# mims-harvard/GNNDelete

Measured on AMD Instinct MI355X. Metric: Del-op train iters/sec, higher is better.
Workload: dtype f32; 1 GPU; synth-collab GCN 2-layer, 5.0% IN edge deletion, full-graph Del step (both_layerwise, mse_mean); num_nodes=235868, in_dim=128, hidden_dim=128, out_dim=64, train_edges_undirected=2122296, df_edges=53057, sdf_edges=1602188, spmm_nnz=1838056, S1=178921, S2=188697, hip_graph=True, matrix_products=fp32 matrix instruction (v_mfma_f32_32x32x2_f32), parallelism=single, ranks_seen=1

## Files before the change

### gnndelete_amd/_lib.py

```python
import ctypes
import os
import re

_HERE = os.path.dirname(os.path.abspath(__file__))
LIB_PATH = os.environ.get('GNNDELETE_HIP_LIB') or os.path.join(_HERE, 'lib', 'libgnndelete_hip.so')
HEADER_PATH = os.path.join(os.path.dirname(_HERE), 'include', 'gnndelete_hip.h')

_i32, _i64, _f32, _f64, _p = ctypes.c_int32, ctypes.c_int64, ctypes.c_float, ctypes.c_double, ctypes.c_void_p

ABI_VERSION = 9

PROTOTYPES = {
    'gd_abi_version': (ctypes.c_int, []),
    'gd_last_error_string': (ctypes.c_char_p, []),
    'gd_build_source_hash': (ctypes.c_char_p, []),
    'gd_matrix_split': (ctypes.c_int, []),
    'gd_set_matrix_split': (ctypes.c_int, [ctypes.c_int]),
    'gd_csr_from_coo_workspace': (_i64, [_i32, _i64]),
    'gd_csr_from_coo': (ctypes.c_int, [_p, _p, _i64, _i32, _p, _p, _p, _p, _p, _i64, _p]),
    'gd_gcn_norm_f32': (ctypes.c_int, [_p, _p, _i32, _p, _p]),
    'gd_spmm_csr_f32': (ctypes.c_int, [_p, _p, _p, _p, _i64, _p, _i64, _p, _f32, _i32, _i32, _p]),
    'gd_spmm_csr_balanced_f32': (ctypes.c_int, [_p, _i32, _p, _i32, _p, _p, _p, _i64, _p, _i64, _p, _f32, _p, _p, _i32,
                                                _i32, _i32, _p, _p]),
    'gd_spmm_csr_onepass_f32': (ctypes.c_int, [_p, _i32, _p, _p, _p, _i64, _p, _i64, _p, _f32, _p, _i32, _i32, _i32, _p, _p]),
# ... 6 lines not shown
    'gd_rgcn_conv_f32': (ctypes.c_int, [_p, _p, _p, _p, _p, _p, _i64, _i32, _p, _i32, _i32, _p, _i64, _i32, _i32, _p]),
    'gd_rowpair_loss_f32': (ctypes.c_int, [_i32, _p, _i64, _p, _p, _i64, _p, _i32, _i32, _p, _p, _i64, _p]),
    'gd_random_walk': (ctypes.c_int, [_p, _p, _i32, _p, _i32, _i32, ctypes.c_uint64, _p, _p]),
    'gd_negative_edges': (ctypes.c_int, [_p, _i64, _i64, ctypes.c_uint64, _p, _i64, _p, _i64, _p]),
    'gd_rank_counts_f32': (ctypes.c_int, [_p, _i64, _p, _i64, _p, _p, _p]),
    'gd_subset_rank_workspace': (_i64, [_i64, _i64]),
    'gd_subset_rank_metrics': (ctypes.c_int, [_p, _p, _p, _p, _p, _i64, _i64, _i64, _i64, _i64, _p, _p, _p, _i64, _p]),
    'gd_subset_rank_metrics_drawn': (ctypes.c_int, [_p, _p, _p, _p, ctypes.c_uint64, ctypes.c_uint64, _i64, _i64, _i64, _i64, _p, _p, _p, _i64, _p]),
    'gd_subset_draw': (ctypes.c_int, [ctypes.c_uint64, ctypes.c_uint64, _i64, _i64, _i64, _p, _i64, _p]),
    'gd_rgcn_tile_kl': (ctypes.c_int32, [_i32, _i32, _i32, _i32]),
    'gd_rgcn_pack_weight_f32': (ctypes.c_int, [_p, _i32, _i32, _i32, _i32, _i32, _p, _p]),
    'gd_rgcn_wave_covers': (ctypes.c_int32, [_i32, _i32, _i32]),
    'gd_rgcn_wave_conv_f32': (ctypes.c_int, [_p, _i32, _i32, _p, _i32, _p, _p, _p, _p, _i64, _i32, _p, _i32, _p, _i64, _i32, _i32, _i32, _p]),
    'gd_rgcn_tile_conv_f32': (ctypes.c_int, [_p, _p, _p, _p, _p, _p, _p, _i32, _p, _i64, _i32, _p, _i32, _i32, _p, _i64, _i32,
                                             _i32, _p, _p, _i32, _p, _p]),
    'gd_rgcn_mean_f32': (ctypes.c_int, [_p, _p, _p, _i64, _p, _i64, _i32, _i32, _i32, _p]),
    'gd_gat_aggregate_f32': (ctypes.c_int, [_p, _p, _p, _p, _p, _i64, _p, _i64, _p, _p, _f32, _i32, _i32, _p]),
    'gd_gat_aggregate_bwd_f32': (ctypes.c_int, [_p, _p, _p, _p, _p, _p, _p, _p, _p, _i64, _p, _i64, _p, _i64,
                                                _p, _p, _p, _f32, _i32, _i32, _p]),
    'gd_gat_balanced_scratch': (_i64, [_i32, _i32]),
    'gd_gat_aggregate_balanced_f32': (ctypes.c_int, [_p, _i32, _p, _i32, _i32, _p, _p, _p, _p, _i64, _p, _i64, _p, _p, _p,
                                                     _p, _f32, _i32, _i32, _i32, _p]),
    'gd_gat_edge_grads_balanced_f32': (ctypes.c_int, [_p, _i32, _p, _i32, _p, _p, _p, _p, _p, _p, _i64, _p, _i64, _p,
                                                      _p, _p, _p, _f32, _i32, _i32, _p, _p]),
    'gd_row_dots_f32': (ctypes.c_int, [_p, _i64, _i32, _i32, _p, _p, _p, _p, _p]),
    'gd_gat_transpose_edges_f32': (ctypes.c_int, [_p, _p, _p, _i32, _p, _p, _p]),
    'gd_rank1_add2_f32': (ctypes.c_int, [_p, _i64, _i32, _i32, _p, _p, _p, _p, _p]),
    'gd_segment_sum_f32': (ctypes.c_int, [_p, _p, _p, _i32, _p, _p]),
    'gd_rows_gemm_f32': (ctypes.c_int, [_p, _i64, _p, _i32, _p, _i32, _i32, _i32, _p, _i32, _p, _i64, _p, _p]),
    'gd_rows_gather_gemm_f32': (ctypes.c_int, [_p, _i64, _i64, _p, _i32, _p, _i32, _i32, _p, _i32, _p, _i64, _p]),
    'gd_rows_gemm_wgrad_workspace': (_i64, [_i32, _i32, _i32]),
    'gd_rows_gemm_ws_covers': (ctypes.c_int, [_i32, _i32, _i32]),
    'gd_rows_gemm_accumulate_f32': (ctypes.c_int, [_p, _i64, _p, _i32, _p, _i32, _i32, _i32, _p, _i64, _p]),
    'gd_rows_gemm_select_f32': (ctypes.c_int, [_p, _p, _p, _i64, _p, _i32, _p, _i32, _i32, _i32, _p, _i32, _p, _i64, _p]),
    'gd_rows_gemm_select_chain_covers': (ctypes.c_int, [_i32, _i32, _i32, _i32, _i32]),
    'gd_rows_gemm_select_chain_f32': (ctypes.c_int, [_p, _i64, _p, _i32, _p, _p, _p, _i64, _p, _i64, _p, _i32, _p, _i32, _i32, _i32,
                                                     _p, _i64, _p]),
    'gd_rows_gemm_dots_f32': (ctypes.c_int, [_p, _p, _p, _i64, _p, _i32, _i32, _i32, _p, _i32, _p, _i64, _p, _i32, _p, _p, _p, _p,
                                             _p]),
    'gd_rows_gemm_signs_f32': (ctypes.c_int, [_p, _i64, _p, _i32, _p, _i32, _i32, _i32, _p, _i32, _p, _i64, _p, _p, _p]),
    'gd_rows_gemm_gated_f32': (ctypes.c_int, [_p, _i64, _p, _i32, _p, _i32, _i32, _i32, _p, _p, _i64, _p]),
    'gd_gate_rows_f32': (ctypes.c_int, [_p, _i64, _p, _i32, _p, _i32, _p, _i64, _p]),
    'gd_rows_gemm_gated_rank1_f32': (ctypes.c_int, [_p, _i64, _p, _i32, _p, _i32, _i32, _i32, _p, _p, _p, _p, _p, _p, _i64, _p]),
    'gd_rows_gemm_wgrad_f32': (ctypes.c_int, [_p, _i64, _p, _p, _i64, _p, _p, _p, _i32, _i32, _i32, _p, _i32, _p, _p]),
    'gd_induced_subgraph_workspace': (_i64, [_i32]),
    'gd_induced_subgraph': (ctypes.c_int, [_p, _p, _p, _i32, _p, _i32, _p, _i32, _p, _i64, _p, _p, _p, _p, _p, _p, _p, _p, _p,
                                           _p, _i64, _p]),
    'gd_batch_csr_workspace': (_i64, [_i32, _i64]),
    'gd_batch_csr': (ctypes.c_int, [_p, _p, _i64, _i32, _i32, _p, _p, _p, _p, _p, _p, _p, _p, _i64, _p]),
    'gd_batch_loss_terms_workspace': (_i64, [_i32, _i64]),
    'gd_batch_loss_terms': (ctypes.c_int, [_p, _i64, _p, _i64, _i32, _p, _i32, _i32, _f32, _f32, _p, _p, _p, _p, _p, _i64, _p]),
    'gd_rowpair_mse_workspace': (_i64, [_i32]),
    'gd_rowpair_mse_f32': (ctypes.c_int, [_p, _i64, _p, _i64, _i32, _p, _p, _i32, _p, _p, _p, _p, _i64, _i32,
                                          _p, _p, _p]),
    'gd_rowtarget_mse_workspace': (_i64, [_i32]),
    'gd_rowtarget_mse_f32': (ctypes.c_int, [_p, _i64, _p, _i32, _p, _p, _p, _p, _i32, _p, _i64, _p, _p, _p]),
    'gd_rowtarget_mse_pair_covers': (ctypes.c_int32, [_i32, _i32]),
    'gd_rowtarget_mse_pair_f32': (ctypes.c_int, [_p, _i64, _p, _i32, _p, _p, _p, _p, _i32, _p, _i64, _p, _p, _i64, _p, _i32, _p, _p, _p, _p, _i32, _p, _i64, _p, _p]),
    'gd_gemm_f32_workspace': (_i64, [_i32, _i32, _i32]),
    'gd_gemm_f32': (ctypes.c_int, [_p, _i64, _p, _i32, _p, _i32, _i32, _p, _p, _i64, _p, _p]),
    'gd_edge_dot_f32': (ctypes.c_int, [_p, _i64, _i32, _p, _p, _p, _i64, _p, _i64, _p, _p]),
    'gd_edge_dot_bwd_f32': (ctypes.c_int, [_p, _i64, _i32, _p, _p, _p, _i64, _p, _p, _i64, _p, _i64, _p]),
    'gd_rows_gemm_wgrad_adam_f32': (ctypes.c_int, [_p, _i64, _p, _p, _i64, _p, _p, _p, _i32, _i32, _i32, _p, _i32, _p,
                                                   _p, _p, _p, _p, _f64, _f64, _f64, _f64, _p]),
    'gd_rows_gemm_wgrad_blocks': (_i32, [_i32]),
    'gd_rows_gemm_wgrad_loss_f32': (ctypes.c_int, [_p, _i64, _p, _p, _i64, _p, _p, _p, _p, _p, _p, _i32, _i32, _i32, _p, _i32,
                                                   _p, _p, _p, _p, _p, _p, _f64, _f64, _f64, _f64, _p]),
    'gd_del_loss_bwd_blocks': (_i32, [_i32]),
    'gd_del_loss_bwd_f32': (ctypes.c_int, [_p, _i64, _p, _i32, _p, _i32, _p, _p, _p, _p, _p, _i64, _p, _i64, _p, _p]),
    'gd_del_loss_bwd_wgrad_f32': (ctypes.c_int, [_p, _i64, _p, _i32, _p, _i32, _p, _p, _p, _p, _p, _i64, _p, _i64, _p, _p, _p]),
    'gd_del_loss_bwd_wgrad_parts': (ctypes.c_int32, [_i32, _i32]),
    'gd_del_loss_bwd_wgrad_parts_f32': (ctypes.c_int, [_p, _i64, _p, _i32, _p, _i32, _p, _p, _p, _p, _p, _i64, _p, _i64, _p, _p, _i32, _p]),
    'gd_del_loss_fold_wgrad_covers': (ctypes.c_int32, [_i32, _i32, _i32]),
    'gd_del_loss_fold_wgrad_parts_f32': (ctypes.c_int, [_p, _i64, _p, _i32, _p, _i32, _p, _p, _p, _p, _p, _i64, _p, _i32, _p, _p, _p, _i32, _p]),
    'gd_del1_loss_wgrad_covers': (ctypes.c_int32, [_i32, _i32]),
    'gd_del1_loss_wgrad_parts': (ctypes.c_int32, [_i32]),
    'gd_del1_chain_loss_wgrad_f32': (ctypes.c_int, [_p, _i64, _p, _i32, _p, _i32, _p, _i64, _p, _p, _p, _p, _p, _p, _i64, _i32, _p, _p, _p, _p, _p, _p, _p, _i32, _p]),
    'gd_del1_chain_fold_covers': (ctypes.c_int32, [_i32, _i32, _i32]),
    'gd_del1_chain_fold_loss_wgrad_f32': (ctypes.c_int, [_p, _i64, _p, _i32, _p, _p, _i32, _p, _i64, _p, _p, _p, _p, _p, _p, _i64, _i32, _p, _p,
                                                         _p, _p, _i32, _p]),
    'gd_layer1_fold_f32': (ctypes.c_int, [_p, _p, _p, _p, _p, _p]),
    'gd_step_tail_fold1_f32': (ctypes.c_int, [_p, _p, _i32, _i32, _i32, _p, _p, _p, _p, _p, _p, _p, _p, _p, _i32, _i32, _i32, _p, _p, _p, _p,
                                              _f64, _f64, _f64, _f64, _p, _i32, _p, _i32, _p, _i32, _p, _p, _p, _p]),
    'gd_del1_loss_wgrad_f32': (ctypes.c_int, [_p, _i64, _p, _i32, _p, _i32, _p, _i64, _p, _p, _p, _p, _p, _p, _i64, _p, _p, _i32, _p]),
    'gd_rowtarget_mse_blocks': (_i32, [_i32]),
    'gd_rowfold_loss_blocks': (_i32, [_i32]),
    'gd_rowfold_loss_f32': (ctypes.c_int, [_i32, _p, _i64, _p, _i32, _i32, _p, _p, _p, _p, _i32, _p, _i64, _p, _p]),
    'gd_rowfold_kld_scale_f32': (ctypes.c_int, [_p, _i32, _f32, _f32, _f32, _f32, _p, _p, _i32, _i32, _p, _i64, _p, _p]),
    'gd_loss_finalize_f32': (ctypes.c_int, [_p, _i32, _p, _i32, _p, _p, _i32, _p, _p, _p]),
    'gd_pairs_sigmoid_mse_workspace': (_i64, [_i32, _i32]),
    'gd_pairs_sigmoid_mse_f32': (ctypes.c_int, [_p, _i64, _p, _i32, _i32, _p, _i64, _f32, _p, _p, _p, _p]),
    'gd_edgeprob_dec_workspace': (_i64, [_i64, _i32]),
    'gd_edgeprob_dec_f32': (ctypes.c_int, [_p, _i64, _i64, _i32, _p, _i64, _p, _i64, _i64, _f32, _p, _p, _p, _p, _p, _p, _p]),
    'gd_edge_incidence_workspace': (_i64, [_i64, _i64]),
    'gd_edge_incidence': (ctypes.c_int, [_p, _p, _i64, _i64, _p, _p, _p, _p, _i64, _p]),
    'gd_edge_incidence_fixed_bytes': (_i64, [_i64, _i64]),
    'gd_edge_incidence_fixed': (ctypes.c_int, [_p, _p, _i64, _i64, _p, _i64, _p, _i64, _p]),
    'gd_edge_incidence_update_workspace': (_i64, [_i64, _i64]),
    'gd_edge_incidence_update': (ctypes.c_int, [_p, _p, _p, _i64, _i64, _i64, _p, _p, _p, _p, _i64, _p]),
    'gd_rows_add_f32': (ctypes.c_int, [_p, _i64, _i64, _p, _i32, _p, _i64, _f32, _i32, _p]),
    'gd_edgeprob_record_f32': (ctypes.c_int, [_p, _p, _f32, _f32, _p, _i32, _p, _p]),
    'gd_edgeprob_batch_loss_workspace': (_i64, [_i64, _i64, _i32]),
    'gd_edgeprob_batch_loss_f32': (ctypes.c_int, [_p, _i64, _i64, _p, _i64, _i64, _i32, _p, _i64, _p, _i64, _i64, _p, _p, _i64, _f32, _f32,
                                                  _p, _i64, _p, _p, _p, _p, _p, _p, _p, _i64, _p, _p]),
    'gd_edge_bce_workspace': (_i64, [_i64, _i32]),
    'gd_edge_bce_f32': (ctypes.c_int, [_p, _i64, _i64, _i32, _p, _i64, _i64, _p, _i64, _i64, _f32, _p, _p, _p, _p, _p, _p, _p]),
    'gd_col_sum_workspace': (_i64, [_i64, _i32]),
    'gd_col_sum_f32': (ctypes.c_int, [_p, _i64, _i64, _i32, _p, _p, _p, _p, _p, _p]),
    'gd_row_nll_workspace': (_i64, [_i64, _i32]),
    'gd_row_nll_f32': (ctypes.c_int, [_p, _i64, _i64, _i32, _i32, _p, _i64, _p, _f32, _p, _i64, _p, _p, _p]),
    'gd_eval_edge_scores_workspace': (_i64, [_i64, _i32]),
    'gd_eval_edge_scores_f32': (ctypes.c_int, [_p, _i64, _i64, _i32, _p, _p, _i64, _i64, _i64, _i64, _p, _p, _p, _p, _p]),
    'gd_eval_triple_scores_workspace': (_i64, [_i64, _i32]),
    'gd_eval_triple_scores_f32': (ctypes.c_int, [_p, _i64, _i64, _i32, _p, _i64, _i64, _p, _p, _p, _i64, _i64, _i64, _i64, _p, _p, _p, _p, _p]),
    'gd_row_nll_eval_workspace': (_i64, [_i64, _i32]),
    'gd_row_nll_eval_f32': (ctypes.c_int, [_p, _i64, _i64, _i32, _p, _i64, _p, _p, _p, _p, _p]),
    'gd_adam_at_f32': (ctypes.c_int, [_p, _p, _p, _p, _p, _i64, _f64, _f64, _f64, _f64, _p]),
    'gd_adam_f32': (ctypes.c_int, [_p, _p, _p, _p, _p, _i64, _f64, _f64, _f64, _f64, _p]),
    'gd_segment_softmax_f32': (ctypes.c_int, [_p, _p, _i32, _p, _p]),
    'gd_segment_softmax_bwd_f32': (ctypes.c_int, [_p, _p, _p, _i32, _p, _p]),
    'gd_rowpair_dot_f32': (ctypes.c_int, [_p, _i64, _p, _p, _i64, _p, _i64, _i32, _p, _p]),
    'gd_spmm_csr_onepass_aux_f32': (ctypes.c_int, [_p, _i32, _p, _p, _p, _p, _i64, _p, _i64, _p, _i32, _i32, _i32, _p, _p]),
    'gd_typed_wgrad_f32': (ctypes.c_int, [_p, _i32, _p, _p, _p, _p, _i64, _p, _i64, _i32, _i32, _i32, _p, _p]),
    'gd_typed_edge_dot_f32': (ctypes.c_int, [_p, _p, _p, _i64, _p, _i64, _p, _i64, _p, _i32, _i32, _i32, _p, _p]),
    'gd_comm_unique_id': (ctypes.c_int, [_p]),
    'gd_comm_init': (ctypes.c_int, [_p, _i32, _i32, ctypes.POINTER(ctypes.c_void_p)]),
    'gd_comm_destroy': (ctypes.c_int, [_p]),
    'gd_allreduce_f32': (ctypes.c_int, [_p, _i64, _p, _p]),
    'gd_exchange_rows_f32': (ctypes.c_int, [_p, _p, _p, _p, _i32, _i32, _p, _p]),
}

_lib = None


class GnnDeleteHipError(RuntimeError):
    pass


def declared_symbols():
    with open(HEADER_PATH) as f:
        text = re.sub(r'/\*.*?\*/', '', f.read(), flags=re.S)
    return sorted(set(re.findall(r'\b(gd_[a-z0-9_]+)\s*\(', text)))


def _sources_hash():
    from .source_hash import source_files, source_hash
    return source_hash() if all(os.path.exists(f) for f in source_files()) and os.path.isdir(os.path.join(_HERE, 'csrc')) else None


def build_stamp():
    return lib().gd_build_source_hash().decode(), _sources_hash()


def lib():
    global _lib
    if _lib is None:
        if not os.path.exists(LIB_PATH):
            raise GnnDeleteHipError(
                f'{LIB_PATH} is missing: the HIP extension is not built. Run '
                '`python -c "import __graft_entry__ as g; g.build()"` (or `make -C gnndelete_amd/csrc`). '
                'There is no CPU fallback.')
        import torch
        handle = ctypes.CDLL(LIB_PATH)
        for name, (res, args) in PROTOTYPES.items():
            fn = getattr(handle, name)
            fn.restype, fn.argtypes = res, args
# ... 24 lines not shown
```

### gnndelete_amd/csrc/rows_gemm.hip

```cpp
#include "common.h"

namespace gd {

using f32x16 = __attribute__((ext_vector_type(16))) float;
using bf16x8 = __attribute__((ext_vector_type(8))) __bf16;
using bf16x2 = __attribute__((ext_vector_type(2))) __bf16;
using f32x2 = __attribute__((ext_vector_type(2))) float;
using u32x4v = __attribute__((ext_vector_type(4))) uint32_t;

__device__ inline void split8(const float4 a, const float4 b, bf16x8 (&s)[3]) {
  const f32x2 v[4] = {{a.x, a.y}, {a.z, a.w}, {b.x, b.y}, {b.z, b.w}};
  u32x4v p[3];
#pragma unroll
  for (int i = 0; i < 4; ++i) {
    f32x2 r = v[i];
#pragma unroll
    for (int q = 0; q < 3; ++q) {
      const uint32_t w = __builtin_bit_cast(uint32_t, __builtin_convertvector(r, bf16x2));
      p[q][i] = w;
      if (q < 2) {
        f32x2 h;
        h[0] = __builtin_bit_cast(float, w << 16);
        h[1] = __builtin_bit_cast(float, w & 0xffff0000u);
        r = r - h;
      }
    }
  }
#pragma unroll
  for (int q = 0; q < 3; ++q) s[q] = __builtin_bit_cast(bf16x8, p[q]);
}

constexpr int kWgradMaxRows = 1024;

constexpr int kGemmThreads = 512;

struct RowDots { const float* u1; const float* u2; float* o1; float* o2; };

template <int NT, int MODE, bool SEL = false, int NP = 0, int KC = 0, bool QUEUE = false, bool GATHER = false>
__global__ __launch_bounds__(QUEUE ? 1024 : kGemmThreads, (NP && KC) ? 2 : 4) void rows_gemm_mfma_kernel(
    const float* in, int64_t ld_in, const int32_t* __restrict__ idx, int32_t n_sel,
    const float* __restrict__ w, int32_t d_in, int32_t trans_w, const float* __restrict__ bias, int32_t relu_in,
    float* out, int64_t ld_out, float* __restrict__ save_in, const uint32_t* __restrict__ gate_bits,
    uint32_t* __restrict__ sign_out, const float* in_alt, const uint8_t* __restrict__ sel, RowDots dots,
    const int64_t* __restrict__ gidx, int32_t n_in) {
  static_assert(!GATHER || (MODE == 0 && !SEL && !QUEUE), "the gathering row map is built for the plain product");
  extern __shared__ __attribute__((aligned(16))) float wl[];
  constexpr int d_out = 32 * NT;
  constexpr int kGemmThreads = QUEUE ? 1024 : gd::kGemmThreads;
  constexpr int kWaves = kGemmThreads / 64;
  static_assert(!QUEUE || (NP == 0 && KC == 0), "the tile queue is built for the fp32 form");
  const int tid = threadIdx.x;
  const int lane = tid & 63;
  const int wave = tid >> 6;

  constexpr int NTP = NT == 3 ? 4 : NT;
  bf16x8* const wimg = reinterpret_cast<bf16x8*>(wl);
  const int pstride = (d_in >> 3) * d_out;
  if (NP) {
    for (int e = tid; e < pstride; e += kGemmThreads) {
      const int kg = e / d_out, n = e - kg * d_out;
      float v[8];
#pragma unroll
      for (int c = 0; c < 8; ++c) v[c] = trans_w ? w[(int64_t)n * d_in + 8 * kg + c] : w[(int64_t)(8 * kg + c) * d_out + n];
      bf16x8 pc[3];
      split8(make_float4(v[0], v[1], v[2], v[3]), make_float4(v[4], v[5], v[6], v[7]), pc);
      const int off = ((((kg >> 2) * 2 + (kg & 1)) * NT + (n >> 5)) * 2 + ((kg >> 1) & 1)) * 32 + (n & 31);
#pragma unroll
      for (int q = 0; q < 3; ++q) wimg[q * pstride + off] = pc[q];
    }
  }
  constexpr int kFill = 8;
  for (int e0 = tid; !NP && e0 < d_in * 32; e0 += kGemmThreads * kFill) {
    float v[kFill][NTP];
#pragma unroll
    for (int u = 0; u < kFill; ++u) {
      const int e = min(e0 + u * kGemmThreads, d_in * 32 - 1);
      const int k = e >> 5, r = e & 31;
#pragma unroll
      for (int t = 0; t < NTP; ++t)
        v[u][t] = t < NT ? (trans_w ? w[(int64_t)(32 * t + r) * d_in + k] : w[(int64_t)k * d_out + 32 * t + r]) : 0.f;
    }
#pragma unroll
    for (int u = 0; u < kFill; ++u) {
// ... 499 lines not shown
    float p = 0.f;
    for (int s = s_begin; s < s_end; ++s) {
      const int64_t ra = a_idx ? a_idx[s] : s, rg = g_idx ? g_idx[s] : s;
      float gg = g[rg * ld_g + j];
      if (relu_mask) gg = relu_mask[rg * ld_g + j] > 0.f ? gg : 0.f;
      if (g_add) gg += g_add[rg * ld_g + j];
      p = fmaf(a[ra * ld_a + i], gg, p);
    }
    dst[e] = p;
  }
}

__global__ __launch_bounds__(256) void wgrad_reduce_kernel(const float* __restrict__ partials, int32_t n_part,
                                                           int32_t n_elem, int32_t accumulate,
                                                           float* __restrict__ dw) {
  __shared__ float4 red[16][16];
  const int v = threadIdx.x & 15, slice = threadIdx.x >> 4;
  const int e4 = blockIdx.x * 16 + v;
  const int n4 = n_elem >> 2;
  float4 s0 = f4_zero(), s1 = f4_zero(), s2 = f4_zero(), s3 = f4_zero();
  if (e4 < n4) {
    int b = slice;
    for (; b + 48 < n_part; b += 64) {
      const float4 p0 = reinterpret_cast<const float4*>(partials + (int64_t)b * n_elem)[e4];
      const float4 p1 = reinterpret_cast<const float4*>(partials + (int64_t)(b + 16) * n_elem)[e4];
      const float4 p2 = reinterpret_cast<const float4*>(partials + (int64_t)(b + 32) * n_elem)[e4];
      const float4 p3 = reinterpret_cast<const float4*>(partials + (int64_t)(b + 48) * n_elem)[e4];
      s0 = f4_add(s0, p0); s1 = f4_add(s1, p1); s2 = f4_add(s2, p2); s3 = f4_add(s3, p3);
    }
    for (; b < n_part; b += 16) s0 = f4_add(s0, reinterpret_cast<const float4*>(partials + (int64_t)b * n_elem)[e4]);
  }
  red[slice][v] = f4_add(f4_add(s0, s1), f4_add(s2, s3));
  __syncthreads();
  if (slice == 0 && e4 < n4) {
    float4 t = accumulate ? reinterpret_cast<float4*>(dw)[e4] : f4_zero();
#pragma unroll
    for (int i = 0; i < 16; ++i) t = f4_add(t, red[i][v]);
    reinterpret_cast<float4*>(dw)[e4] = t;
  }
}

__global__ __launch_bounds__(256) void wgrad_reduce_adam_kernel(const float* __restrict__ partials, int32_t n_part,
                                                                int32_t n_elem, int32_t accumulate,
                                                                float* __restrict__ dw, float* __restrict__ param,
                                                                float* __restrict__ m, float* __restrict__ v,
                                                                const int32_t* __restrict__ iter, double lr, double beta1,
                                                                double beta2, double eps) {
  __shared__ float4 red[16][16];
  const int vv = threadIdx.x & 15, slice = threadIdx.x >> 4;
  const int e4 = blockIdx.x * 16 + vv;
  const int n4 = n_elem >> 2;
  float4 s0 = f4_zero(), s1 = f4_zero(), s2 = f4_zero(), s3 = f4_zero();
  if (e4 < n4) {
    int b = slice;
    for (; b + 48 < n_part; b += 64) {
      const float4 p0 = reinterpret_cast<const float4*>(partials + (int64_t)b * n_elem)[e4];
      const float4 p1 = reinterpret_cast<const float4*>(partials + (int64_t)(b + 16) * n_elem)[e4];
      const float4 p2 = reinterpret_cast<const float4*>(partials + (int64_t)(b + 32) * n_elem)[e4];
      const float4 p3 = reinterpret_cast<const float4*>(partials + (int64_t)(b + 48) * n_elem)[e4];
      s0 = f4_add(s0, p0); s1 = f4_add(s1, p1); s2 = f4_add(s2, p2); s3 = f4_add(s3, p3);
    }
    for (; b < n_part; b += 16) s0 = f4_add(s0, reinterpret_cast<const float4*>(partials + (int64_t)b * n_elem)[e4]);
  }
  red[slice][vv] = f4_add(f4_add(s0, s1), f4_add(s2, s3));
  __syncthreads();
  if (slice == 0 && e4 < n4) {
    float4 t4 = accumulate ? reinterpret_cast<float4*>(dw)[e4] : f4_zero();
#pragma unroll
    for (int i = 0; i < 16; ++i) t4 = f4_add(t4, red[i][vv]);
    reinterpret_cast<float4*>(dw)[e4] = t4;
    const AdamScalars sc = adam_scalars(lr, beta1, beta2, eps, *iter + 1);
    float4 p4 = reinterpret_cast<float4*>(param)[e4], m4 = reinterpret_cast<float4*>(m)[e4],
           v4 = reinterpret_cast<float4*>(v)[e4];
    adam_update(p4.x, m4.x, v4.x, t4.x, sc);
    adam_update(p4.y, m4.y, v4.y, t4.y, sc);
    adam_update(p4.z, m4.z, v4.z, t4.z, sc);
    adam_update(p4.w, m4.w, v4.w, t4.w, sc);
    reinterpret_cast<float4*>(param)[e4] = p4;
    reinterpret_cast<float4*>(m)[e4] = m4;
    reinterpret_cast<float4*>(v)[e4] = v4;
  }
}

struct TailJob {
  const float* partials; int32_t n_part, n_elem, accumulate;
  float* dw; float* param; float* m; float* v;
};
struct TailFin {
  const float* p1; int32_t n1; const float* p2; int32_t n2;
  float* hist; int32_t capacity; int32_t* pos; int32_t* iter; int32_t* arrive;
};

__device__ __forceinline__ int32_t tail_check_in(const TailFin& fin) {
  int32_t t = atomicAdd(fin.iter, 0);
  asm volatile("" : "+v"(t));
  atomicAdd(fin.arrive + (t < 0 ? 1 : 0), 1);
  return t + 1;
}

__device__ __forceinline__ void tail_job_block(const TailJob& j, int blk, const TailFin& fin, float4 (*red)[16], int32_t* t_sh, double lr,
                                               double beta1, double beta2, double eps) {
  const int tid = threadIdx.x;
  if (tid == 0) *t_sh = tail_check_in(fin);
  const int vv = tid & 15, slice = tid >> 4;
  const int e4 = blk * 16 + vv;
  const int n4 = j.n_elem >> 2;
  float4 s0 = f4_zero(), s1 = f4_zero(), s2 = f4_zero(), s3 = f4_zero();
  if (e4 < n4) {
    int b = slice;
    for (; b + 48 < j.n_part; b += 64) {
      const float4 p0 = reinterpret_cast<const float4*>(j.partials + (int64_t)b * j.n_elem)[e4];
      const float4 p1 = reinterpret_cast<const float4*>(j.partials + (int64_t)(b + 16) * j.n_elem)[e4];
      const float4 p2 = reinterpret_cast<const float4*>(j.partials + (int64_t)(b + 32) * j.n_elem)[e4];
      const float4 p3 = reinterpret_cast<const float4*>(j.partials + (int64_t)(b + 48) * j.n_elem)[e4];
      s0 = f4_add(s0, p0); s1 = f4_add(s1, p1); s2 = f4_add(s2, p2); s3 = f4_add(s3, p3);
    }
    for (; b < j.n_part; b += 16) s0 = f4_add(s0, reinterpret_cast<const float4*>(j.partials + (int64_t)b * j.n_elem)[e4]);
  }
  red[slice][vv] = f4_add(f4_add(s0, s1), f4_add(s2, s3));
  __syncthreads();
  if (slice == 0 && e4 < n4) {
    float4 t4 = j.accumulate ? reinterpret_cast<float4*>(j.dw)[e4] : f4_zero();
#pragma unroll
    for (int i = 0; i < 16; ++i) t4 = f4_add(t4, red[i][vv]);
    reinterpret_cast<float4*>(j.dw)[e4] = t4;
    const AdamScalars sc = adam_scalars(lr, beta1, beta2, eps, *t_sh);
    float4 p4 = reinterpret_cast<float4*>(j.param)[e4], m4 = reinterpret_cast<float4*>(j.m)[e4],
           v4 = reinterpret_cast<float4*>(j.v)[e4];
    adam_update(p4.x, m4.x, v4.x, t4.x, sc);
    adam_update(p4.y, m4.y, v4.y, t4.y, sc);
    adam_update(p4.z, m4.z, v4.z, t4.z, sc);
    adam_update(p4.w, m4.w, v4.w, t4.w, sc);
    reinterpret_cast<float4*>(j.param)[e4] = p4;
    reinterpret_cast<float4*>(j.m)[e4] = m4;
    reinterpret_cast<float4*>(j.v)[e4] = v4;
  }
}

__device__ __forceinline__ void tail_finalize_block(const TailFin& fin, float (*fred)[256], int n_wait) {
  const int tid = threadIdx.x;
  float a = 0.f, b = 0.f, c = 0.f, d = 0.f;
  for (int i = tid; i < fin.n1; i += 256) { a += fin.p1[2 * i]; b += fin.p1[2 * i + 1]; }
  for (int i = tid; i < fin.n2; i += 256) { c += fin.p2[2 * i]; d += fin.p2[2 * i + 1]; }
  fred[0][tid] = a; fred[1][tid] = b; fred[2][tid] = c; fred[3][tid] = d;
  __syncthreads();
  for (int off = 128; off > 0; off >>= 1) {
    if (tid < off) {
#pragma unroll
      for (int q = 0; q < 4; ++q) fred[q][tid] += fred[q][tid + off];
    }
    __syncthreads();
  }
  if (tid < 4) fin.hist[(int64_t)(*fin.pos) * 4 + tid] = fred[tid][0];
  __syncthreads();
  if (tid == 0) {
    while (atomicAdd(fin.arrive, 0) < n_wait) __builtin_amdgcn_s_sleep(8);
    *fin.arrive = 0;
    *fin.pos = (*fin.pos + 1) % fin.capacity;
    atomicAdd(fin.iter, 1);
  }
}

__global__ __launch_bounds__(256) void step_tail_kernel(TailJob j1, TailJob j2, TailFin fin, double lr, double beta1, double beta2,
                                                        double eps) {
  __shared__ float4 red[16][16];
  __shared__ float fred[4][256];
  __shared__ int32_t t_sh;
  const int nb1 = (j1.n_elem / 4 + 15) / 16, nb2 = (j2.n_elem / 4 + 15) / 16;
  if ((int)blockIdx.x < nb1 + nb2) {
    const bool first = (int)blockIdx.x < nb1;
    tail_job_block(first ? j1 : j2, first ? blockIdx.x : blockIdx.x - nb1, fin, red, &t_sh, lr, beta1, beta2, eps);
    return;
  }
  tail_finalize_block(fin, fred, nb1 + nb2);
}

__device__ __forceinline__ void fold1_column(const float* w1s, const float* __restrict__ b1, const float* wd_col, int c, float* scr,
                                             float* __restrict__ wf, float* __restrict__ bf) {
  const int tid = threadIdx.x, i = tid & 127, hf = tid >> 7;
  float acc = 0.f;
#pragma unroll 16
  for (int j = 64 * hf; j < 64 * hf + 64; ++j) acc = fmaf(w1s[j * 129 + i], wd_col[j], acc);
  scr[tid] = acc;
  __syncthreads();
  if (tid < 128) wf[(int64_t)tid * 128 + c] = scr[tid] + scr[tid + 128];
  __syncthreads();
  scr[tid] = tid < 128 ? b1[tid] * wd_col[tid] : 0.f;
  __syncthreads();
  for (int off = 64; off > 0; off >>= 1) {
    if (tid < off) scr[tid] += scr[tid + off];
    __syncthreads();
  }
  if (tid == 0) bf[c] = scr[0];
  __syncthreads();
}

__device__ __forceinline__ void fold1_fetch_w1(const float* __restrict__ w1, float4 (&r)[16]) {
#pragma unroll
  for (int it = 0; it < 16; ++it) r[it] = reinterpret_cast<const float4*>(w1)[threadIdx.x + 256 * it];
}
__device__ __forceinline__ void fold1_store_w1(const float4 (&r)[16], float* w1s) {
#pragma unroll
  for (int it = 0; it < 16; ++it) {
    const int e = threadIdx.x + 256 * it;
    float* dst = w1s + (e >> 5) * 129 + (e & 31) * 4;
    dst[0] = r[it].x; dst[1] = r[it].y; dst[2] = r[it].z; dst[3] = r[it].w;
  }
}

__global__ __launch_bounds__(256) void layer1_fold_kernel(const float* __restrict__ w1, const float* __restrict__ b1, const float* __restrict__ wd,
                                                          float* __restrict__ wf, float* __restrict__ bf) {
  extern __shared__ __attribute__((aligned(16))) float w1s[];
  __shared__ float wd_col[128];
  __shared__ float scr[256];
  const int c = blockIdx.x;
  float4 w1r[16];
  fold1_fetch_w1(w1, w1r);
  if (threadIdx.x < 128) wd_col[threadIdx.x] = wd[(int64_t)threadIdx.x * 128 + c];
  fold1_store_w1(w1r, w1s);
  __syncthreads();
  fold1_column(w1s, b1, wd_col, c, scr, wf, bf);
}

struct TailFold1 { const float* colsum; const float* w1; const float* b1; float* wf; float* bf; };

__global__ __launch_bounds__(256) void step_tail_fold1_kernel(TailJob j1, TailJob j2, TailFin fin, TailFold1 fo, double lr, double beta1,
                                                              double beta2, double eps) {
  extern __shared__ __attribute__((aligned(16))) float w1s[];
  __shared__ float4 red[16][16];
  __shared__ float fred[4][256];
  __shared__ float gcol[128], wd_col[128];
  __shared__ int32_t t_sh;
  constexpr int D = 128;
  const int nb2 = (j2.n_elem / 4 + 15) / 16;
  const int tid = threadIdx.x;
  if ((int)blockIdx.x >= D + nb2) { tail_finalize_block(fin, fred, D + nb2); return; }
  if ((int)blockIdx.x >= D) { tail_job_block(j2, blockIdx.x - D, fin, red, &t_sh, lr, beta1, beta2, eps); return; }
  const int c = blockIdx.x;
  if (tid == 0) t_sh = tail_check_in(fin);
  float4 w1r[16];
  fold1_fetch_w1(fo.w1, w1r);
  {
    const int vv = tid & 31, slice = tid >> 5;
    const float4* src = reinterpret_cast<const float4*>(j1.partials + (int64_t)c * D) + vv;
    const int64_t pitch4 = (int64_t)D * D / 4;
    float4 sa[8];
#pragma unroll
    for (int q = 0; q < 8; ++q) sa[q] = f4_zero();
    int b = slice;
    for (; b + 56 < j1.n_part; b += 64) {
      float4 pv[8];
#pragma unroll
      for (int q = 0; q < 8; ++q) pv[q] = src[(b + 8 * q) * pitch4];
#pragma unroll
      for (int q = 0; q < 8; ++q) sa[q] = f4_add(sa[q], pv[q]);
    }
    for (; b < j1.n_part; b += 8) sa[0] = f4_add(sa[0], src[b * pitch4]);
    float4* const red8 = &red[0][0];
    red8[slice * 32 + vv] = f4_add(f4_add(f4_add(sa[0], sa[1]), f4_add(sa[2], sa[3])), f4_add(f4_add(sa[4], sa[5]), f4_add(sa[6], sa[7])));
    float cs = 0.f;
    for (int q = tid; q < j1.n_part; q += 256) cs += fo.colsum[(int64_t)q * D + c];
    fred[0][tid] = cs;
    fold1_store_w1(w1r, w1s);
    __syncthreads();
    if (tid < 32) {
      float4 t4 = red8[tid];
#pragma unroll
      for (int i = 1; i < 8; ++i) t4 = f4_add(t4, red8[i * 32 + tid]);
      reinterpret_cast<float4*>(gcol)[tid] = t4;
    }
    for (int off = 128; off > 0; off >>= 1) {
      if (tid < off) fred[0][tid] += fred[0][tid + off];
      __syncthreads();
    }
  }
  {
    const int j = tid & 127, hf = tid >> 7;
    float acc = 0.f;
#pragma unroll 16
    for (int i = 64 * hf; i < 64 * hf + 64; ++i) acc = fmaf(w1s[j * 129 + i], gcol[i], acc);
    fred[1][tid] = acc;
    __syncthreads();
    if (tid < D) {
      const float g = fmaf(fo.b1[tid], fred[0][0], fred[1][tid] + fred[1][tid + 128]);
      const int64_t e = (int64_t)tid * D + c;
      j1.dw[e] = g;
      const AdamScalars sc = adam_scalars(lr, beta1, beta2, eps, t_sh);
      float pv = j1.param[e], mv = j1.m[e], vv = j1.v[e];
      adam_update(pv, mv, vv, g, sc);
      j1.param[e] = pv; j1.m[e] = mv; j1.v[e] = vv;
      wd_col[tid] = pv;
    }
    __syncthreads();
  }
  fold1_column(w1s, fo.b1, wd_col, c, fred[2], fo.wf, fo.bf);
}

__global__ __launch_bounds__(256) void wgrad_reduce_scalar_kernel(const float* __restrict__ partials, int32_t n_part,
                                                                  int32_t n_elem, int32_t accumulate,
                                                                  float* __restrict__ dw) {
  const int e = blockIdx.x * 256 + threadIdx.x;
  if (e >= n_elem) return;
  float s = accumulate ? dw[e] : 0.f;
  for (int b = 0; b < n_part; ++b) s += partials[(int64_t)b * n_elem + e];
  dw[e] = s;
}

static inline void wgrad_geometry(int32_t n_sel, int* n_blocks, int* rows_per_block) {
  int nb = (n_sel + 127) / 128;
  if (nb > 512) nb = 512;
  if (nb < (n_sel + kWgradMaxRows - 1) / kWgradMaxRows) nb = (n_sel + kWgradMaxRows - 1) / kWgradMaxRows;
  if (nb < 1) nb = 1;
  int rpb = (n_sel + nb - 1) / nb;
  rpb = (rpb + 31) / 32 * 32;
  if (rpb < 32) rpb = 32;
  *n_blocks = (n_sel + rpb - 1) / rpb;
  if (*n_blocks < 1) *n_blocks = 1;
  *rows_per_block = rpb;
}

}

static int rows_gemm_impl(const float* in, int64_t ld_in, const int32_t* idx, int32_t n_sel, const float* w,
                          int32_t d_in, int32_t d_out, int32_t trans_w, const float* bias, int32_t relu_in,
                          const uint32_t* gate_bits, uint32_t* sign_out, float* out, int64_t ld_out,
                          float* save_in, void* stream, const float* in_alt = nullptr, const uint8_t* sel = nullptr,
                          gd::RowDots dots = gd::RowDots{nullptr, nullptr, nullptr, nullptr}, const int64_t* gidx = nullptr,
                          int32_t n_in = 0) {
  using namespace gd;
  GD_REQUIRE(!sel || (in_alt && aligned16(in_alt) && in_alt != out && !gate_bits && !sign_out), GD_E_NULL,
             "gd_rows_gemm_select_f32: bad in_alt");
  GD_REQUIRE(in && w && out, GD_E_NULL, "gd_rows_gemm_f32: null pointer");
  GD_REQUIRE(n_sel >= 0 && d_in > 0 && d_out > 0 && ld_in >= d_in && ld_out >= d_out, GD_E_DIM,
             "gd_rows_gemm_f32: bad dims n_sel=%d d_in=%d d_out=%d", n_sel, d_in, d_out);
  GD_REQUIRE(in != out || d_in == d_out, GD_E_DIM, "gd_rows_gemm_f32: in-place needs d_in == d_out");
  GD_REQUIRE(!(gate_bits && sign_out), GD_E_DIM, "gd_rows_gemm_f32: gate and sign output are exclusive");
  if (n_sel == 0) return GD_OK;
  if (!gidx) {
    const int rc = rows_gemm_ws_try(in, ld_in, idx, n_sel, w, d_in, d_out, trans_w, bias, relu_in, gate_bits, sign_out, out, ld_out,
                                    save_in, stream, in_alt, sel, dots.u1, dots.u2, dots.o1, dots.o2);
    if (rc != 1) return rc;
  }
  hipStream_t s = (hipStream_t)stream;
  size_t lds = (size_t)d_in * 32 * (d_out / 32 == 3 ? 4 : d_out / 32) * sizeof(float);
  const int np = matrix_split();
  const bool mfma_ok = (d_out % 32 == 0) && d_out <= 128 && (d_in % 32 == 0) && lds <= 64 * 1024 && aligned16(in) &&
                       (ld_in % 4 == 0) && (!save_in || aligned16(save_in)) && aligned16(out) && (ld_out % 4 == 0) &&
                       (!bias || aligned16(bias));
  if (mfma_ok) {
    const int n_tiles = (n_sel + 31) / 32;
    int grid = (n_tiles + 7) / 8;
    static const int grid_cap = [] { const char* e = getenv("GD_ROWS_GEMM_GRID"); return e && atoi(e) > 0 ? atoi(e) : 512; }();
    if (grid > grid_cap) grid = grid_cap;
    static const bool spread_on = [] { const char* e = getenv("GD_ROWS_GEMM_SPREAD"); return !(e && atoi(e) == 0); }();
    if (spread_on && grid < ws_cu_count()) grid = n_tiles < ws_cu_count() ? n_tiles : ws_cu_count();
    const int kc_split = (np && (d_in == 64 || d_in == 128) && d_out >= 96) ? d_in / 32 : 0;
    const bool narrow_split = np && !kc_split && d_out == 64 && d_in == 128;
    if (kc_split || narrow_split) {
      lds = (size_t)3 * d_in * d_out * 2;
      if (grid > grid_cap / 2 && lds > 80 * 1024) grid = grid_cap / 2;
    }
    static const bool queue_on = [] { const char* e = getenv("GD_ROWS_GEMM_QUEUE"); return !(e && atoi(e) == 0); }();
    const bool use_queue = queue_on && !kc_split && !narrow_split && n_tiles >= 16 * 256 && !gidx;
    if (use_queue && grid > ws_cu_count()) grid = ws_cu_count();
#define GD_RG_KERNEL(NT, MODE, SELV, NPV, KCV, GV)                                                                 \
  do {                                                                                                            \
    if (use_queue && !NPV && !GV) {                                                                                 \
      auto kq = rows_gemm_mfma_kernel<NT, MODE, SELV, 0, 0, true>;                                                \
              \
      static const hipError_t onceq = hipFuncSetAttribute((const void*)kq, hipFuncAttributeMaxDynamicSharedMemorySize, 64 * 1024 + 64); \
      GD_REQUIRE(onceq == hipSuccess, -(int)onceq, "gd_rows_gemm_f32: cannot raise the LDS limit of the tile-queue kernel"); \
      hipLaunchKernelGGL(kq, dim3(grid), dim3(1024), lds, s, in, ld_in, idx, n_sel, w, d_in, trans_w,             \
                         bias, relu_in, out, ld_out, save_in, gate_bits, sign_out, in_alt, sel, dots, gidx, n_in); \
      break;                                                                                                      \
    }                                                                                                             \
    auto kern = rows_gemm_mfma_kernel<NT, MODE, SELV, NPV, KCV, false, GV>;                                            \
    if (NPV && lds > 64 * 1024) {                                                                                 \
      static const hipError_t once = hipFuncSetAttribute((const void*)kern, hipFuncAttributeMaxDynamicSharedMemorySize, 160 * 1024); \
// ... 373 lines not shown
```

### gnndelete_amd/csrc/spmm.hip

```cpp
#include <stdlib.h>
#include <string.h>

#include "common.h"

namespace gd {

template <int LPR, int VPL, bool MEAN>
__global__ __launch_bounds__(256) void spmm_vec_kernel(const int32_t* __restrict__ rowptr,
                                                       const int32_t* __restrict__ col,
                                                       const float* __restrict__ val,
                                                       const float* __restrict__ x, int64_t ldx,
                                                       float* __restrict__ y, int64_t ldy,
                                                       const float* __restrict__ bias, float self_coef,
                                                       int32_t n_rows, int32_t x_rows_mod, int32_t d4) {
  constexpr int G = kWave / LPR;
  const int lane = threadIdx.x & 63;
  const int row = blockIdx.x * 4 + (threadIdx.x >> 6);
  if (row >= n_rows) return;
  const int g = lane / LPR;
  const int li = lane % LPR;
  const int start = rowptr[row];
  const int end = rowptr[row + 1];

  float4 acc[VPL];
#pragma unroll
  for (int v = 0; v < VPL; ++v) acc[v] = f4_zero();

  for (int base = start; base < end; base += kWave) {
    const int k = base + lane;
    const bool live = k < end;
    const int c = live ? col[k] : 0;
    const float w = live ? (val ? val[k] : 1.0f) : 0.0f;
    const int cnt = min(kWave, end - base);
    const int trips = (cnt + G - 1) / G;

    for (int it = 0; it < trips; ++it) {
      const int j = it * G + g;
      const int cj = __shfl(c, j);
      const float wj = __shfl(w, j);
      const float4* xr = reinterpret_cast<const float4*>(x + (int64_t)cj * ldx);
#pragma unroll
      for (int v = 0; v < VPL; ++v) {
        const int vec = li + v * LPR;
        if (vec < d4) acc[v] = f4_fma(wj, xr[vec], acc[v]);
      }
    }
  }
#pragma unroll
  for (int v = 0; v < VPL; ++v) {
#pragma unroll
    for (int off = LPR; off < kWave; off <<= 1) acc[v] = f4_add(acc[v], f4_shfl_xor(acc[v], off));
  }
  if (g != 0) return;
  const float scale = MEAN ? (end > start ? 1.0f / (float)(end - start) : 0.0f) : 1.0f;
  const int self_row = x_rows_mod > 0 ? row % x_rows_mod : row;
#pragma unroll
  for (int v = 0; v < VPL; ++v) {
    const int vec = li + v * LPR;
    if (vec >= d4) continue;
    float4 o = acc[v];
    if (MEAN) {
      o.x *= scale; o.y *= scale; o.z *= scale; o.w *= scale;
    } else {
      if (self_coef != 0.0f) {
        const float4 s = reinterpret_cast<const float4*>(x + (int64_t)self_row * ldx)[vec];
        o = f4_fma(self_coef, s, o);
      }
      if (bias) o = f4_add(o, reinterpret_cast<const float4*>(bias)[vec]);
    }
    reinterpret_cast<float4*>(y + (int64_t)row * ldy)[vec] = o;
  }
}

template <int LPR, int VPL, int U, bool EXACT, bool ADDR32, bool AUX = false, bool NOVAL = false>
__device__ __forceinline__ void spmm_persist_body(const int4* __restrict__ items, int32_t n_items,
                                                  const int32_t* __restrict__ xcd_bounds,
                                                  const int32_t* __restrict__ col, const float* __restrict__ val,
                                                  const float* __restrict__ x, int64_t ldx, float* __restrict__ y,
                                                  int64_t ldy, const float* __restrict__ bias, float self_coef,
                                                  const float* __restrict__ xs, float* __restrict__ scratch, int32_t d4,
                                                  int32_t nnz, const int32_t* __restrict__ perm = nullptr,
                                                  const float2* __restrict__ aux = nullptr, float* __restrict__ aux_sum = nullptr) {
  constexpr int G = kWave / LPR;
  constexpr int kXcd = 8;
  const int lane = threadIdx.x & 63;
  const int g = lane / LPR, li = lane % LPR;
// ... 192 lines not shown
      }
      d0 = d1;
      d1 = uniform(dv);
      continue;
    }
#pragma unroll
    for (int v = 0; v < VPL; ++v) acc[v] = f4_group_sum<LPR>(acc[v]);
    if (AUX && slot == -1 && row >= 0) {
      const float s1 = wave_sum(lane < d0.end - d0.start ? a_raw : 0.f);
      if (lane == 0) aux_sum[row] = s1;
    }
    if (slot == -2) {
      const int wave = threadIdx.x >> 6;
      if (g == 0) {
#pragma unroll
        for (int v = 0; v < VPL; ++v) grp_red[wave][li + v * LPR] = acc[v];
      }
      if (AUX && lane == 0) grp_aux[wave] = a_sum;
      __syncthreads();
      if (AUX && wave == 0 && lane == 0 && row >= 0) aux_sum[row] = ((grp_aux[0] + grp_aux[1]) + grp_aux[2]) + grp_aux[3];
      if (wave == 0 && g == 0) {
        char* ob = reinterpret_cast<char*>(y + (int64_t)row * ldy);
        const char* sb = reinterpret_cast<const char*>(xs + (int64_t)row * ldx);
#pragma unroll
        for (int v = 0; v < VPL; ++v) {
          if (!EXACT && li + v * LPR >= d4) continue;
          const int e = li + v * LPR;
          float4 o = f4_add(f4_add(f4_add(grp_red[0][e], grp_red[1][e]), grp_red[2][e]), grp_red[3][e]);
          if (self_coef != 0.0f) o = f4_fma(self_coef, *reinterpret_cast<const float4*>(sb + lo[v]), o);
          if (bias) o = f4_add(o, *reinterpret_cast<const float4*>(bb + lo[v]));
          *reinterpret_cast<float4*>(ob + lo[v]) = o;
        }
      }
      __syncthreads();
    } else if (g == 0 && row >= 0) {
      char* ob = whole ? reinterpret_cast<char*>(y + (int64_t)row * ldy)
                       : reinterpret_cast<char*>(scratch + (int64_t)slot * d4 * 4);
      const char* sb = reinterpret_cast<const char*>(xs + (int64_t)row * ldx);
#pragma unroll
      for (int v = 0; v < VPL; ++v) {
        if (!EXACT && li + v * LPR >= d4) continue;
        float4 o = acc[v];
        if (self && !self_in_acc) o = f4_fma(self_coef, *reinterpret_cast<const float4*>(sb + lo[v]), o);
        *reinterpret_cast<float4*>(ob + lo[v]) = o;
      }
    }
    d0 = d1;
    d1 = uniform(dv);
  }
}

template <int LPR, int VPL, int U, bool EXACT, bool ADDR32, bool NOVAL = false>
__global__ __launch_bounds__(256) void spmm_persist_kernel(const int4* __restrict__ items, int32_t n_items,
                                                           const int32_t* __restrict__ xcd_bounds,
                                                           const int32_t* __restrict__ col,
                                                           const float* __restrict__ val,
                                                           const float* __restrict__ x, int64_t ldx,
                                                           float* __restrict__ y, int64_t ldy,
                                                           const float* __restrict__ bias, float self_coef,
                                                           const float* __restrict__ xs,
                                                           float* __restrict__ scratch, int32_t d4, int32_t nnz) {
  spmm_persist_body<LPR, VPL, U, EXACT, ADDR32, false, NOVAL>(items, n_items, xcd_bounds, col, val, x, ldx, y, ldy, bias, self_coef, xs,
                                                              scratch, d4, nnz);
}

template <int LPR>
__global__ __launch_bounds__(256) void spmm_persist_aux_kernel(const int4* __restrict__ items, int32_t n_items,
                                                               const int32_t* __restrict__ xcd_bounds,
                                                               const int32_t* __restrict__ col, const float* __restrict__ val,
                                                               const float* __restrict__ x, int64_t ldx, float* __restrict__ y,
                                                               int64_t ldy, const float* __restrict__ bias, float self_coef,
                                                               const float* __restrict__ xs, float* __restrict__ scratch, int32_t d4,
                                                               int32_t nnz, const int32_t* __restrict__ perm,
                                                               const float2* __restrict__ aux, float* __restrict__ aux_sum) {
  spmm_persist_body<LPR, 1, 4, true, true, true>(items, n_items, xcd_bounds, col, val, x, ldx, y, ldy, bias, self_coef, xs, scratch, d4,
                                                 nnz, perm, aux, aux_sum);
}

typedef float f32x4_t __attribute__((ext_vector_type(4)));
#ifndef GD_SPMM_WIDE_GRID_CAP
#define GD_SPMM_WIDE_GRID_CAP 8192
#endif

__global__ __launch_bounds__(256) __attribute__((amdgpu_waves_per_eu(8, 8))) void spmm_wide_kernel(
    const int4* __restrict__ items, int32_t n_items, const int32_t* __restrict__ xcd_bounds, const int32_t* __restrict__ colt,
    const float* __restrict__ val, const float* __restrict__ x, int64_t ldx, float* __restrict__ y, int64_t ldy,
    const float* __restrict__ bias, float self_coef, const float* __restrict__ xs, int32_t nnz) {
  constexpr int kXcd = 8, U = 4;
  constexpr int kSrcMask = (1 << 24) - 1;
  const int lane = threadIdx.x & 63;
  const int g = lane >> 4, li = lane & 15;
  const int xcd = blockIdx.x % kXcd;
  const int stride = (gridDim.x / kXcd) * 4;
  const int wx = (blockIdx.x / kXcd) * 4 + (threadIdx.x >> 6);
  const int i0 = xcd_bounds[xcd], i1 = xcd_bounds[xcd + 1];
  if ((i0 | i1) & 3) __builtin_trap();
  const uint32_t lo = 16u * (uint32_t)li;
  const uint32_t pitch_b = (uint32_t)ldx * 4u, pitch_y = (uint32_t)ldy * 4u;
  const char* xb = reinterpret_cast<const char*>(x);

  int i = __builtin_amdgcn_readfirstlane(i0 + wx);
  if (i >= i1) return;
  int4 d0 = items[i], d1 = items[min(i + stride, i1 - 1)];
  int kk = min(d0.y + lane, nnz - 1);
  int c = colt[kk];
  float w = val ? val[kk] : 1.0f;
  __shared__ float4 grp_red[4][16];
  __shared__ float4 bias_s[16];
  if (threadIdx.x < 16) bias_s[threadIdx.x] = bias ? reinterpret_cast<const float4*>(bias)[threadIdx.x] : f4_zero();
  __syncthreads();
  for (; i < i1; i += stride) {
    const int row = d0.x, slot = d0.w;
    const int c_now = c;
    const float w_now = w;
    const int4 d2 = items[min(i + 2 * stride, i1 - 1)];
    kk = min(d1.y + lane, nnz - 1);
    c = colt[kk];
    w = val ? val[kk] : 1.0f;
    if (slot != -2) {
      const int nr = -slot - 15;
      const int cnt = d0.z - d0.y;
      const float w_cur = lane < cnt ? w_now : 0.f;
      const int trips = (cnt + 3) >> 2;
      const int last4 = 4 * cnt - 4, end4 = 4 * cnt;
      const float4 bv = bias_s[li];
      f32x4_t a0 = {bv.x, bv.x, bv.x, bv.x}, a1 = {bv.y, bv.y, bv.y, bv.y}, a2 = {bv.z, bv.z, bv.z, bv.z}, a3 = {bv.w, bv.w, bv.w, bv.w};
      auto fetch = [&](int t, float4& xv, float& av) {
        const int j4 = 16 * t + 4 * g;
        const int cs = __builtin_amdgcn_ds_bpermute(min(j4, last4), c_now);
        const float wj = __int_as_float(__builtin_amdgcn_ds_bpermute(min(j4, end4), __float_as_int(w_cur)));
        av = ((uint32_t)cs >> 24) == (uint32_t)li ? wj : 0.f;
        const uint32_t ro = __umul24((uint32_t)(cs & kSrcMask), pitch_b);
        xv = *reinterpret_cast<const float4*>(xb + (ro + lo));
      };
      auto mma = [&](float av, const float4& xv) {
        a0 = __builtin_amdgcn_mfma_f32_16x16x4f32(av, xv.x, a0, 0, 0, 0);
        a1 = __builtin_amdgcn_mfma_f32_16x16x4f32(av, xv.y, a1, 0, 0, 0);
        a2 = __builtin_amdgcn_mfma_f32_16x16x4f32(av, xv.z, a2, 0, 0, 0);
        a3 = __builtin_amdgcn_mfma_f32_16x16x4f32(av, xv.w, a3, 0, 0, 0);
      };
      int t0 = 0;
      for (; t0 + U <= trips; t0 += U) {
        float4 xv[U];
        float av[U];
#pragma unroll
        for (int u = 0; u < U; ++u) fetch(t0 + u, xv[u], av[u]);
        __builtin_amdgcn_sched_barrier(0);
#pragma unroll
        for (int u = 0; u < U; ++u) mma(av[u], xv[u]);
      }
      const int rem = trips - t0;
      if (rem == 1) {
        float4 xv;
        float av;
        fetch(t0, xv, av);
        mma(av, xv);
      } else if (rem == 2) {
        float4 xv[2];
        float av[2];
        fetch(t0, xv[0], av[0]);
        fetch(t0 + 1, xv[1], av[1]);
        mma(av[0], xv[0]);
        mma(av[1], xv[1]);
      } else if (rem == 3) {
        float4 xv[3];
        float av[3];
        fetch(t0, xv[0], av[0]);
        fetch(t0 + 1, xv[1], av[1]);
        fetch(t0 + 2, xv[2], av[2]);
        mma(av[0], xv[0]);
        mma(av[1], xv[1]);
        mma(av[2], xv[2]);
      }
      const uint32_t r0 = (uint32_t)(row + 4 * g);
#pragma unroll
      for (int j = 0; j < 4; ++j) {
        if (4 * g + j < nr) {
          float4 o = make_float4(a0[j], a1[j], a2[j], a3[j]);
          if (self_coef != 0.0f)
            o = f4_fma(self_coef, *reinterpret_cast<const float4*>(reinterpret_cast<const char*>(xs) + (__umul24(r0 + j, pitch_b) + lo)), o);
          *reinterpret_cast<float4*>(reinterpret_cast<char*>(y) + (__umul24(r0 + j, pitch_y) + lo)) = o;
        }
      }
    } else {
      int base = d0.y;
      int c_cur = c_now;
      float w_raw = w_now;
      float4 acc = f4_zero();
      for (;;) {
        const int cnt = min(kWave, d0.z - base);
        const float w_cur = lane < cnt ? w_raw : 0.f;
        const int trips = (cnt + 3) >> 2;
        const int last4 = 4 * cnt - 4, end4 = 4 * cnt;
        auto fetch = [&](int t, float4& xv, float& wj) {
          const int j4 = 16 * t + 4 * g;
          const int cs = __builtin_amdgcn_ds_bpermute(min(j4, last4), c_cur);
          wj = __int_as_float(__builtin_amdgcn_ds_bpermute(min(j4, end4), __float_as_int(w_cur)));
          const uint32_t ro = __umul24((uint32_t)(cs & kSrcMask), pitch_b);
          xv = *reinterpret_cast<const float4*>(xb + (ro + lo));
        };
        int t0 = 0;
        for (; t0 + U <= trips; t0 += U) {
          float4 xv[U];
          float wj[U];
#pragma unroll
          for (int u = 0; u < U; ++u) fetch(t0 + u, xv[u], wj[u]);
#pragma unroll
          for (int u = 0; u < U; ++u) acc = f4_fma(wj[u], xv[u], acc);
        }
        const int rem = trips - t0;
        if (rem == 1) {
          float4 xv;
          float wj;
          fetch(t0, xv, wj);
          acc = f4_fma(wj, xv, acc);
        } else if (rem == 2) {
          float4 xv[2];
          float wj[2];
          fetch(t0, xv[0], wj[0]);
          fetch(t0 + 1, xv[1], wj[1]);
          acc = f4_fma(wj[1], xv[1], f4_fma(wj[0], xv[0], acc));
        } else if (rem == 3) {
          float4 xv[3];
          float wj[3];
          fetch(t0, xv[0], wj[0]);
          fetch(t0 + 1, xv[1], wj[1]);
          fetch(t0 + 2, xv[2], wj[2]);
          acc = f4_fma(wj[2], xv[2], f4_fma(wj[1], xv[1], f4_fma(wj[0], xv[0], acc)));
        }
        base += kWave;
        if (base >= d0.z) break;
        const int k2 = min(base + lane, nnz - 1);
        c_cur = colt[k2];
        w_raw = val ? val[k2] : 1.0f;
      }
      acc = f4_group_sum<16>(acc);
      const int wave = threadIdx.x >> 6;
      if (g == 0) grp_red[wave][li] = acc;
      __syncthreads();
      if (wave == 0 && g == 0) {
        float4 o = f4_add(f4_add(f4_add(grp_red[0][li], grp_red[1][li]), grp_red[2][li]), grp_red[3][li]);
        if (self_coef != 0.0f)
          o = f4_fma(self_coef, *reinterpret_cast<const float4*>(reinterpret_cast<const char*>(xs) + (__umul24((uint32_t)row, pitch_b) + lo)), o);
        if (bias) o = f4_add(o, bias_s[li]);
        *reinterpret_cast<float4*>(reinterpret_cast<char*>(y) + (__umul24((uint32_t)row, pitch_y) + lo)) = o;
      }
      __syncthreads();
    }
    d0 = d1;
    d1 = d2;
  }
}

__global__ __launch_bounds__(256) void spmm_fixup_kernel(const int4* __restrict__ split, int32_t n_split,
                                                         const float* __restrict__ scratch,
                                                         const float* __restrict__ x, int64_t ldx,
                                                         float* __restrict__ y, int64_t ldy,
                                                         const float* __restrict__ bias, float self_coef,
                                                         int32_t d4) {
  const int lane = threadIdx.x & 63;
  const int i = blockIdx.x * 4 + (threadIdx.x >> 6);
  if (i >= n_split) return;
  const int4 sp = split[i];
  const int row = sp.x, slot0 = sp.y, n = sp.z;
  for (int vec = lane; vec < d4; vec += kWave) {
    float4 o = f4_zero();
    const float4* sp4 = reinterpret_cast<const float4*>(scratch + (int64_t)slot0 * d4 * 4) + vec;
    int s = 0;
    for (; s + 4 <= n; s += 4) {
      const float4 p0 = sp4[(int64_t)s * d4], p1 = sp4[(int64_t)(s + 1) * d4], p2 = sp4[(int64_t)(s + 2) * d4],
                   p3 = sp4[(int64_t)(s + 3) * d4];
      o = f4_add(f4_add(f4_add(f4_add(o, p0), p1), p2), p3);
    }
    for (; s < n; ++s) o = f4_add(o, sp4[(int64_t)s * d4]);
    if (self_coef != 0.0f) o = f4_fma(self_coef, reinterpret_cast<const float4*>(x + (int64_t)row * ldx)[vec], o);
    if (bias) o = f4_add(o, reinterpret_cast<const float4*>(bias)[vec]);
    reinterpret_cast<float4*>(y + (int64_t)row * ldy)[vec] = o;
  }
}

template <bool MEAN>
__global__ __launch_bounds__(256) void spmm_scalar_kernel(const int32_t* __restrict__ rowptr,
                                                          const int32_t* __restrict__ col,
                                                          const float* __restrict__ val,
                                                          const float* __restrict__ x, int64_t ldx,
                                                          float* __restrict__ y, int64_t ldy,
                                                          const float* __restrict__ bias, float self_coef,
                                                          int32_t n_rows, int32_t x_rows_mod, int32_t d) {
  const int lane = threadIdx.x & 63;
  const int row = blockIdx.x * 4 + (threadIdx.x >> 6);
  if (row >= n_rows) return;
  const int start = rowptr[row], end = rowptr[row + 1];
  const int self_row = x_rows_mod > 0 ? row % x_rows_mod : row;
  for (int c0 = 0; c0 < d; c0 += kWave) {
    const int cc = c0 + lane;
    float acc = 0.f;
    for (int k = start; k < end; ++k) {
      const float w = val ? val[k] : 1.0f;
      if (cc < d) acc = fmaf(w, x[(int64_t)col[k] * ldx + cc], acc);
    }
    if (cc < d) {
      if (MEAN) {
        acc = end > start ? acc / (float)(end - start) : 0.f;
      } else {
        if (self_coef != 0.0f) acc = fmaf(self_coef, x[(int64_t)self_row * ldx + cc], acc);
        if (bias) acc += bias[cc];
      }
      y[(int64_t)row * ldy + cc] = acc;
    }
  }
}

__global__ __launch_bounds__(256) void gcn_norm_kernel(const int32_t* __restrict__ rowptr,
                                                       const int32_t* __restrict__ col, int32_t n_rows,
                                                       float* __restrict__ val) {
  const int lane = threadIdx.x & 63;
  const int row = blockIdx.x * 4 + (threadIdx.x >> 6);
  if (row >= n_rows) return;
  const int start = rowptr[row], end = rowptr[row + 1];
  const float di = 1.0f / sqrtf((float)(end - start));
  for (int k = start + lane; k < end; k += kWave) {
    const int c = col[k];
    const float dj = 1.0f / sqrtf((float)(rowptr[c + 1] - rowptr[c]));
    val[k] = dj * di;
  }
}

template <bool MEAN>
static int launch_spmm(const int32_t* rowptr, const int32_t* col, const float* val, const float* x,
                       int64_t ldx, float* y, int64_t ldy, const float* bias, float self_coef,
                       int32_t n_rows, int32_t x_rows_mod, int32_t d, hipStream_t s) {
  if (n_rows == 0 || d == 0) return GD_OK;
  const dim3 grid((n_rows + 3) / 4), block(256);
  const bool vec_ok = (d % 4 == 0) && (ldx % 4 == 0) && (ldy % 4 == 0) && aligned16(x) && aligned16(y) &&
                      (!bias || aligned16(bias)) && d <= 1024;
  if (!vec_ok) {
// ... 70 lines not shown
#define GD_ITEMS_LAUNCH(LPR, VPL, EXACT, A32)                                                                        \
  hipLaunchKernelGGL((spmm_persist_kernel<LPR, VPL, ((64 / (64 / LPR)) >= 4 ? 4 : (64 / (64 / LPR))), EXACT, A32>), \
                     grid, block, 0, s, it, n_items, xcd_bounds, col, val, x, ldx, y, ldy, bias, self_coef, xs, scratch, \
                     d4, nnz)
#define GD_ITEMS_CASE(LPR, VPL)                                                                                    \
  do {                                                                                                             \
    if (d4 == LPR * VPL) {                                                                                         \
      if (addr32) GD_ITEMS_LAUNCH(LPR, VPL, true, true);                                                           \
      else GD_ITEMS_LAUNCH(LPR, VPL, true, false);                                                                 \
    } else {                                                                                                       \
      if (addr32) GD_ITEMS_LAUNCH(LPR, VPL, false, true);                                                          \
      else GD_ITEMS_LAUNCH(LPR, VPL, false, false);                                                                \
    }                                                                                                              \
  } while (0)
  if (d4 == 16 && addr32 && val == nullptr) {
    const char* form = getenv("GD_SPMM_D64_FORM");
    if (form && !strncmp(form, "16x1", 4) && strchr(form, 'n') != nullptr) {
      hipLaunchKernelGGL((spmm_persist_kernel<16, 1, 4, true, true, true>), grid, block, 0, s, it, n_items, xcd_bounds, col, val, x,
                         ldx, y, ldy, bias, self_coef, xs, scratch, d4, nnz);
      return launched("spmm_persist");
    }
  }
  if (d4 <= 1) GD_ITEMS_CASE(1, 1);
  else if (d4 <= 2) GD_ITEMS_CASE(2, 1);
  else if (d4 <= 4) GD_ITEMS_CASE(4, 1);
  else if (d4 <= 8) GD_ITEMS_CASE(8, 1);
  else if (d4 <= 16) GD_ITEMS_CASE(16, 1);
  else if (d4 <= 32) GD_ITEMS_CASE(32, 1);
  else if (d4 <= 64) GD_ITEMS_CASE(64, 1);
  else if (d4 <= 128) GD_ITEMS_CASE(64, 2);
  else GD_ITEMS_CASE(64, 4);
#undef GD_ITEMS_CASE
#undef GD_ITEMS_LAUNCH
  return launched("spmm_persist");
}
}

extern "C" int gd_spmm_csr_balanced_f32(const int32_t* items, int32_t n_items, const int32_t* split, int32_t n_split,
                                        const int32_t* col, const float* val, const float* x, int64_t ldx, float* y,
                                        int64_t ldy, const float* bias, float self_coef, const float* x_self,
                                        float* scratch, int32_t d, int32_t nnz, int32_t x_rows,
                                        const int32_t* xcd_bounds, void* stream) {
  using namespace gd;
  GD_REQUIRE(items && col && x && y, GD_E_NULL, "gd_spmm_csr_balanced_f32: null pointer");
  GD_REQUIRE(n_split == 0 || (split && scratch), GD_E_NULL, "gd_spmm_csr_balanced_f32: split rows need scratch");
  GD_REQUIRE(n_items >= 0 && n_split >= 0 && d > 0 && d % 4 == 0 && d <= 1024 && ldx % 4 == 0 && ldy % 4 == 0, GD_E_DIM,
             "gd_spmm_csr_balanced_f32: d=%d must be a multiple of 4 (<=1024) with 16-byte row strides", d);
  GD_REQUIRE(aligned16(x) && aligned16(y) && aligned16(items) && (!bias || aligned16(bias)) &&
                 (!scratch || aligned16(scratch)) && (!split || aligned16(split)), GD_E_ALIGN,
             "gd_spmm_csr_balanced_f32: unaligned pointer");
  GD_REQUIRE(x != y, GD_E_DIM, "gd_spmm_csr_balanced_f32: x and y must not alias");
  if (n_items == 0) return GD_OK;
  hipStream_t s = (hipStream_t)stream;
  const int d4 = d / 4;
  const float* xs = x_self ? x_self : x;
  GD_REQUIRE(aligned16(xs) && xs != y, GD_E_ALIGN, "gd_spmm_csr_balanced_f32: bad x_self");
  float* scratch_arg = scratch ? scratch : reinterpret_cast<float*>(const_cast<int32_t*>(items));
  int rc = launch_persist(items, n_items, col, val, x, ldx, y, ldy, bias, self_coef, xs, scratch_arg, d, nnz, x_rows,
                          xcd_bounds, s);
  if (rc || n_split == 0) return rc;
  hipLaunchKernelGGL(spmm_fixup_kernel, dim3((n_split + 3) / 4), dim3(256), 0, s, reinterpret_cast<const int4*>(split),
                     n_split, scratch, xs, ldx, y, ldy, bias, self_coef, d4);
  return launched("spmm_fixup");
}

extern "C" int gd_spmm_csr_onepass_f32(const int32_t* items, int32_t n_items, const int32_t* col, const float* val,
                                       const float* x, int64_t ldx, float* y, int64_t ldy, const float* bias,
                                       float self_coef, const float* x_self, int32_t d, int32_t nnz, int32_t x_rows,
                                       const int32_t* xcd_bounds, void* stream) {
  using namespace gd;
  GD_REQUIRE(col && x && y && xcd_bounds && (items || n_items == 0), GD_E_NULL, "gd_spmm_csr_onepass_f32: null pointer");
  GD_REQUIRE(n_items >= 0 && n_items % 4 == 0 && d > 0 && d % 4 == 0 && d <= 1024 && ldx % 4 == 0 && ldy % 4 == 0, GD_E_DIM,
             "gd_spmm_csr_onepass_f32: d=%d must be a multiple of 4 (<=1024) with 16-byte row strides, n_items a multiple of 4", d);
  GD_REQUIRE(aligned16(x) && aligned16(y) && aligned16(items) && (!bias || aligned16(bias)), GD_E_ALIGN,
             "gd_spmm_csr_onepass_f32: unaligned pointer");
  GD_REQUIRE(x != y, GD_E_DIM, "gd_spmm_csr_onepass_f32: x and y must not alias");
  if (n_items == 0) return GD_OK;
  const float* xs = x_self ? x_self : x;
  GD_REQUIRE(aligned16(xs) && xs != y, GD_E_ALIGN, "gd_spmm_csr_onepass_f32: bad x_self");
  return launch_persist(items, n_items, col, val, x, ldx, y, ldy, bias, self_coef, xs, nullptr, d, nnz, x_rows,
                        xcd_bounds, (hipStream_t)stream);
}

extern "C" int gd_spmm_csr_onepass_wide_f32(const int32_t* items, int32_t n_items, const int32_t* col_tagged, const float* val,
                                            const float* x, int64_t ldx, float* y, int64_t ldy, const float* bias,
                                            float self_coef, const float* x_self, int32_t d, int32_t nnz, int32_t x_rows,
                                            const int32_t* xcd_bounds, void* stream) {
  using namespace gd;
  GD_REQUIRE(col_tagged && x && y && xcd_bounds && (items || n_items == 0), GD_E_NULL, "gd_spmm_csr_onepass_wide_f32: null pointer");
  GD_REQUIRE(n_items >= 0 && n_items % 4 == 0 && d == 64 && ldx % 4 == 0 && ldy % 4 == 0 && ldx >= d && ldy >= d, GD_E_DIM,
             "gd_spmm_csr_onepass_wide_f32: d must be 64 (got %d) with 16-byte row strides, n_items a multiple of 4", d);
  GD_REQUIRE(aligned16(x) && aligned16(y) && aligned16(items) && (!bias || aligned16(bias)), GD_E_ALIGN,
             "gd_spmm_csr_onepass_wide_f32: unaligned pointer");
  GD_REQUIRE(x != y, GD_E_DIM, "gd_spmm_csr_onepass_wide_f32: x and y must not alias");
  GD_REQUIRE(x_rows > 0 && x_rows < (1 << 24) && ldx * 4 < (1 << 24) && ldy * 4 < (1 << 24) &&
                 (int64_t)x_rows * ldx * 4 < (1ll << 32) && (int64_t)x_rows * ldy * 4 < (1ll << 32), GD_E_DIM,
             "gd_spmm_csr_onepass_wide_f32: x and y must be smaller than 4 GiB with row ids and pitches below 2^24");
  if (n_items == 0) return GD_OK;
  const float* xs = x_self ? x_self : x;
  GD_REQUIRE(aligned16(xs) && xs != y, GD_E_ALIGN, "gd_spmm_csr_onepass_wide_f32: bad x_self");
  const char* e = getenv("GD_SPMM_GRID_CAP");
  const int cap_env = e ? atoi(e) : 0;
  const int cap = cap_env > 0 ? cap_env : GD_SPMM_WIDE_GRID_CAP;
  int nblk = (n_items + 3) / 4;
  if (nblk > cap) nblk = cap;
  nblk = (nblk + 7) / 8 * 8;
  hipLaunchKernelGGL(spmm_wide_kernel, dim3(nblk), dim3(256), 0, (hipStream_t)stream, reinterpret_cast<const int4*>(items), n_items,
                     xcd_bounds, col_tagged, val, x, ldx, y, ldy, bias, self_coef, xs, nnz);
  return launched("spmm_wide");
}

extern "C" int gd_spmm_csr_onepass_aux_f32(const int32_t* items, int32_t n_items, const int32_t* col, const int32_t* perm,
                                           const float* aux, const float* x, int64_t ldx, float* y, int64_t ldy, float* aux_sum,
                                           int32_t d, int32_t nnz, int32_t x_rows, const int32_t* xcd_bounds, void* stream) {
  using namespace gd;
  GD_REQUIRE(col && perm && aux && x && y && aux_sum && xcd_bounds && (items || n_items == 0), GD_E_NULL,
             "gd_spmm_csr_onepass_aux_f32: null pointer");
  GD_REQUIRE(n_items >= 0 && n_items % 4 == 0 && (d == 64 || d == 128) && ldx % 4 == 0 && ldy % 4 == 0 && ldx >= d && ldy >= d, GD_E_DIM,
             "gd_spmm_csr_onepass_aux_f32: d must be 64 or 128 (got %d), 16-byte row strides, n_items a multiple of 4", d);
  GD_REQUIRE(aligned16(x) && aligned16(y) && aligned16(items) && (reinterpret_cast<uintptr_t>(aux) & 7u) == 0, GD_E_ALIGN,
             "gd_spmm_csr_onepass_aux_f32: unaligned pointer");
  GD_REQUIRE(x != y, GD_E_DIM, "gd_spmm_csr_onepass_aux_f32: x and y must not alias");
  GD_REQUIRE(x_rows > 0 && x_rows <= (1 << 24) && ldx * 4 < (1 << 24) && ldy * 4 < (1 << 24) &&
                 (int64_t)x_rows * ldx * 4 < (1ll << 32) && (int64_t)x_rows * ldy * 4 < (1ll << 32), GD_E_DIM,
             "gd_spmm_csr_onepass_aux_f32: x and y must be smaller than 4 GiB with row ids and pitches below 2^24");
  if (n_items == 0) return GD_OK;
  int nblk = (n_items + 3) / 4;
  if (nblk > 8192) nblk = 8192;
  nblk = (nblk + 7) / 8 * 8;
  const int4* it = reinterpret_cast<const int4*>(items);
  const float2* a2 = reinterpret_cast<const float2*>(aux);
  if (d == 64)
    hipLaunchKernelGGL((spmm_persist_aux_kernel<16>), dim3(nblk), dim3(256), 0, (hipStream_t)stream, it, n_items, xcd_bounds, col, (const float*)nullptr,
                       x, ldx, y, ldy, (const float*)nullptr, 0.0f, x, (float*)nullptr, d / 4, nnz, perm, a2, aux_sum);
  else
    hipLaunchKernelGGL((spmm_persist_aux_kernel<32>), dim3(nblk), dim3(256), 0, (hipStream_t)stream, it, n_items, xcd_bounds, col, (const float*)nullptr,
                       x, ldx, y, ldy, (const float*)nullptr, 0.0f, x, (float*)nullptr, d / 4, nnz, perm, a2, aux_sum);
  return launched("spmm_persist_aux");
}
```

### gnndelete_amd/engine.py

```python
import os
import warnings
from typing import NamedTuple

import torch

from . import _lib, ops
from ._lib import check, ptr, stream_ptr
from .capture import capture_iterations
from .graph import graph_for
from .nn import GATConv, GCNConv, GINConv, RGCNConv, SAGEConv

LOSS_TYPES = ('both_all', 'both_layerwise', 'only2_layerwise', 'only2_all', 'only1')


class StepFacts(NamedTuple):
    mode: str
    loss_type: str
    family: str
    h: int
    o: int
    s1: int
    s2: int
    folded1: bool
    n_rows1: int
# ... 37 lines not shown
        raw = env.get('GD_' + name.upper())
        if name == 'pad_out':
            try:
                val[name] = default if raw is None else int(raw)
            except ValueError:
                warnings.warn(f'GD_PAD_OUT={raw!r} is not an integer: the class dimension is not padded')
                val[name] = 0
        else:
            val[name] = (raw != '0') if default else (raw == '1')
    return Knobs(**val)


class StepForms(NamedTuple):
    split1: bool
    split2: bool
    out1: bool
    out2: bool
    fuse_loss1: bool
    fuse_l2: bool
    tail: bool
    fuse_wg2: bool
    fuse_del1: bool
    chain1: bool
    out_pair: bool
    rows_only: bool
    rgcn_rows_only: bool
    gat_dots: bool


def plan_step(facts, k):
    (mode, loss_type, family, h, o, s1, s2, folded1, n_rows1, inside1, folded2, n_rows2, inside2, cache_layer1, rows_only_asked,
     closed, w2_mfma, gin_ok, del1_covers, pair_covers) = facts
    mse = family == 'mse'
    mixed_ok = folded1 and folded2 and not k.no_split_loss and not k.no_split
    out2 = not inside2 and mixed_ok and mse and s2 > 0 and o in (32, 64) and n_rows2 > 0 and not k.no_fused_l2
    split2 = (inside2 or out2) and not k.no_split
    fuse_l2 = mse and split2 and folded1 and o in (32, 64) and n_rows2 > 0 and not k.no_fused_l2
    split1 = (not cache_layer1 or k.cache_split) and inside1 and not k.no_split
    loss1_ok = (mse and folded1 and folded2 and loss_type in ('both_layerwise', 'both_all', 'only1') and s1 > 0
                and h in (32, 64, 128) and n_rows1 > 0 and not k.no_fused_loss1)
    out1 = loss1_ok and not inside1 and mixed_ok
    fuse_loss1 = loss1_ok and (inside1 or out1)
    tail = (folded1 and folded2 and s1 > 0 and s2 > 0 and loss_type in ('both_layerwise', 'both_all') and h % 2 == 0 and o % 2 == 0
            and not k.no_step_tail
            and ((fuse_loss1 and fuse_l2) or (h in (32, 64, 128) and o in (32, 64, 128) and not k.tail_fused_only)))
    fuse_wg2 = tail and fuse_l2 and not k.no_fused_wgrad2
    fuse_del1 = tail and fuse_loss1 and split1 and loss_type in ('both_layerwise', 'only1') and del1_covers
    chain1 = (fuse_del1 and loss_type == 'both_layerwise' and h == 128 and o == 64 and k.del1_chain
              and (mode in ('gcn', 'gin') or (mode == 'gat' and w2_mfma and not k.no_gat_rank1_epilogue)))
    out_pair = out1 and out2 and fuse_loss1 and fuse_l2 and loss_type != 'only2_all' and pair_covers and not k.no_loss_pair
    rows_only = (rows_only_asked and (mode in ('gcn', 'gat', 'sage') or gin_ok) and split2 and s2 > 0
                 and not out1 and not out2 and closed)
    return StepForms(split1, split2, out1, out2, fuse_loss1, fuse_l2, tail, fuse_wg2, fuse_del1, chain1, out_pair, rows_only,
                     rows_only_asked and mode == 'rgcn', not k.no_gat_dots)


def read_del2_fold(env=None):
    env = os.environ if env is None else env
    return env.get('GD_DEL2_FOLD') != '0'


def plan_del2_fold(facts, forms, covers, enabled=True):
    return bool(enabled and covers and forms.chain1 and facts.mode in ('gcn', 'gin') and forms.fuse_wg2 and not forms.out2)


def read_layer1_fold(env=None):
    env = os.environ if env is None else env
    return env.get('GD_LAYER1_FOLD') != '0'


def plan_layer1_fold(facts, forms, covers, enabled=True):
    return bool(enabled and covers and forms.chain1 and forms.fuse_del1 and forms.split1 and facts.mode == 'gcn'
                and facts.loss_type == 'both_layerwise' and not facts.cache_layer1 and facts.h == 128)


def read_explicit_chain(env=None):
    env = os.environ if env is None else env
    return env.get('GD_EXPLICIT_CHAIN') != '0'


def plan_explicit_chain(facts, forms, covers, enabled=True, *, fold1, n_explicit):
    return bool(enabled and covers and fold1 and facts.mode == 'gcn' and not forms.rows_only and not facts.cache_layer1
                and facts.h == 128 and facts.o == 64 and n_explicit > 0)


def _loss_coefficients(loss_type, alpha):
    if loss_type in ('both_all', 'both_layerwise', 'only2_layerwise'):
        return alpha, 1.0 - alpha
    return alpha, 1.0


LOSS_FAMILIES = {'mse_mean': ('mse', 'mean'), 'mse_sum': ('mse', 'sum'), 'kld_mean': ('kld', 'mean'), 'kld_sum': ('kld', 'sum'),
                 'cosine_mean': ('cosine', 'mean'), 'cosine_sum': ('cosine', 'sum')}
_ROWFOLD_FAMILY = {'cosine': 0, 'kld': 1}


def fold_row_terms(family, z_ori, rows, tgt, kind, d_valid=None):
    assert family in ('kld', 'cosine'), family
    d = z_ori.shape[1]
    dv = d if d_valid is None else int(d_valid)
    device = z_ori.device
    uniq, inv, c = torch.unique(rows, return_inverse=True, return_counts=True)
    kind_u = torch.zeros(uniq.numel(), dtype=torch.int32, device=device)
    kind_u[inv] = kind.to(torch.int32)
    if uniq.numel() == 0:
        return uniq, torch.zeros(0, d, dtype=torch.float64, device=device), c, kind_u, [0.0, 0.0]
    order = torch.argsort(inv, stable=True)
    o64 = z_ori[tgt[order]][:, :dv].double()
    if family == 'cosine':
        u = o64 / o64.norm(dim=1, keepdim=True).clamp_(min=1e-8)
        tm = torch.segment_reduce(u, 'sum', lengths=c, axis=0)
        k_row = torch.zeros(uniq.numel(), dtype=torch.float64, device=device)
    else:
        t = torch.softmax(o64, 1)
        tm = torch.segment_reduce(t, 'sum', lengths=c, axis=0)
        ent = torch.segment_reduce(torch.special.xlogy(t, t).sum(1), 'sum', lengths=c, axis=0)
        k_row = (ent - torch.special.xlogy(tm, tm / c[:, None].double()).sum(1)).clamp_(min=0.0)
    if dv < d:
        tm = torch.nn.functional.pad(tm, (0, d - dv))
    return uniq, tm, c, kind_u, [float(k_row[kind_u == 0].sum()), float(k_row[kind_u == 1].sum())]


def logged_loss(family, raw_sum, k_const, n):
    v = (raw_sum + k_const) / n
    return 1.0 - torch.exp(-v) if family == 'kld' else v


def _members(idx, n_sel, rows):
    pos = torch.searchsorted(idx, rows)
    return (pos < n_sel) & (idx[pos.clamp(max=n_sel - 1)] == rows), pos


class _LayerTerms:

    def __init__(self, pos_edge, neg_edge, ni_mask, z_ori, coef_r, coef_l, reduction, row_range=None, d_norm=None, family='mse'):
        device = z_ori.device
        self.family = family
        self.d_valid = z_ori.shape[1] if d_norm is None else int(d_norm)
        d = z_ori.shape[1]
        dn = d if d_norm is None else int(d_norm)
        pos, neg = pos_edge.to(device).long(), neg_edge.to(device).long()
        ni_rows = ni_mask.to(device).nonzero().flatten()
        m = pos.shape[1]
        if family != 'mse':
            dn = 1
        self.n_r = (2 * m * dn) if reduction == 'mean' else 1
        self.n_l = (ni_rows.numel() * dn) if reduction == 'mean' else 1
        self.count_r, self.count_l = 2 * m, int(ni_rows.numel())
        w_r, w_l = coef_r / max(self.n_r, 1), coef_l / max(self.n_l, 1)
        rows = torch.cat([pos[0], pos[1], ni_rows])
        tgt = torch.cat([neg[0], neg[1], ni_rows])
        kind = torch.cat([torch.zeros(2 * m, dtype=torch.int32, device=device),
                          torch.ones(ni_rows.numel(), dtype=torch.int32, device=device)])
        mixed = bool(ni_mask.to(device)[pos.flatten()].any()) if m else False
        if row_range is not None:
            mine = (rows >= row_range[0]) & (rows < row_range[1])
            rows, tgt, kind = rows[mine], tgt[mine], kind[mine]
        self.k_const = [0.0, 0.0]
        self.folded = not mixed
        if family != 'mse':
            if mixed:
                raise ValueError(f'the folded {family} loss needs one kind of term per row: a Neighborhood-Influence row of this request is an '
                                 'endpoint of a deleted edge (the autograd loop handles such a request)')
            if row_range is not None:
                raise ValueError(f'the folded {family} loss has no row-partitioned form (its scalar would need an all-reduce in mid-step)')
            uniq, tm, c, kind_u, self.k_const = fold_row_terms(family, z_ori, rows, tgt, kind, self.d_valid)
# ... 294 lines not shown
        lib = _lib.lib()
        if self._out2:
            self.t2.order_inside_first(self.idx2, self.s2)
        if self._out1:
            self.t1.order_inside_first(self.idx1, self.s1)
        self.z1 = torch.empty(n, self.h, **f32)
        self.z2 = torch.empty(n, self.o, **f32)
        self.p2 = torch.empty(n, self.o, **f32) if self._split2 else self.z2
        self.xs2 = None if self._split2 else torch.empty(max(1, self.s2), self.o, **f32)
        self._lp1 = self._lp2 = None
        self._lp1_blocks = self._lp2_blocks = 0
        if self._fuse_l2:
            self._slot2, self._cnt_signed2 = _loss_slots(self.t2, self.idx2, self.s2, dev)
            if self._fuse_wg2:
                self._lp2_blocks = lib.gd_del_loss_bwd_wgrad_parts(self.s2, self.o)
                lp2_size = lib.gd_rows_gemm_wgrad_blocks(self.s2)
            else:
                self._lp2_blocks = lp2_size = lib.gd_del_loss_bwd_blocks(self.s2)
            self._lp2 = torch.zeros(2 * max(1, lp2_size + self.t2.outside_blocks()), **f32)
            self.dz2c = torch.zeros(self.s2, self.o, **f32)
        self.pre1 = torch.empty(n, self.h, **f32) if self._split1 else self.z1
        self._sel1 = m1.to(torch.uint8).contiguous() if self._split1 else None
        self.xs1 = None if self._split1 else torch.empty(max(1, self.s1), self.h, **f32)
        self.dz1 = torch.zeros(n, self.h, **f32)
        if isinstance(conv2, SAGEConv):
            self.dcat = torch.zeros(n, 2 * self.o, **f32)
            self.dz2 = self.dcat[:, self.o:]
        else:
            self.dz2 = torch.zeros(n, self.o, **f32)
        self.dh = torch.zeros(n, self.h, **f32)
        self.z1_pos = torch.zeros(max(1, self.s1), (self.h + 31) // 32, dtype=torch.int32, device=dev)
        self.g1 = torch.zeros_like(self.wd1)
        self.g2 = torch.zeros_like(self.wd2)
        self.sums = torch.zeros(4, **f32)
        self.ws1 = torch.empty(max(1, lib.gd_rows_gemm_wgrad_workspace(self.s1, self.h, self.h)), **f32)
        self.ws2 = torch.empty(max(1, lib.gd_rows_gemm_wgrad_workspace(self.s2, self.o, self.o)), **f32)
        self.iter_ctr = torch.zeros(1, dtype=torch.int32, device=dev)
        self.adam1, self.adam2 = _Adam(self.wd1, lr, iter_ctr=self.iter_ctr), _Adam(self.wd2, lr, iter_ctr=self.iter_ctr)
        self.hist = torch.zeros(history, 4, **f32)
        self.hist_pos = torch.zeros(1, dtype=torch.int32, device=dev)
        self.steps_done = 0
        self._graph = self._graph_k = None
        self._use_graph = use_graph
        self._const_refs = {}
        if self._fuse_loss1:
            self._slot1, self._cnt_signed1 = _loss_slots(self.t1, self.idx1, self.s1, dev)
            self._lp1_blocks = lib.gd_del1_loss_wgrad_parts(self.s1) if self._fuse_del1 else lib.gd_rows_gemm_wgrad_blocks(self.s1)
            self._lp1 = torch.zeros(2 * max(1, lib.gd_rows_gemm_wgrad_blocks(self.s1) + self.t1.outside_blocks()), **f32)
        self._tail_acc = [0, 0]
        self._arrive = torch.zeros(2, dtype=torch.int32, device=dev)
        self._gat_bufs = self._dt2_keep = None
        if self._chain1 and self._mode == 'gat':
            self._gat_bufs = {'dh': torch.zeros(n, self.o, **f32), 'da_src': torch.zeros(n, **f32), 'da_dst': torch.zeros(n, **f32)}
        elif self._chain1:
            self._dt2_keep = torch.zeros(n, self.o, **f32)
        self._fold2 = plan_del2_fold(self.facts, self.forms, lib.gd_del_loss_fold_wgrad_covers(self.s2, self.o, self.h), read_del2_fold())
        self._w2fold = torch.zeros(self.o, self.h, **f32) if self._fold2 else None
        self._fold1 = False
        if self._mode == 'gcn':
            w1_ = conv1.lin.weight
            self._fold1 = plan_layer1_fold(
                self.facts, self.forms,
                tuple(w1_.shape) == (128, 128) and x.shape[1] == 128 and x.dtype == torch.float32
                and bool(lib.gd_del1_chain_fold_covers(self.s1, x.shape[1], self.h)), read_layer1_fold())
        if self._fold1:
            self._w1 = conv1.lin.weight.detach().float().contiguous()
            self._b1 = (conv1.bias.detach().float().contiguous() if conv1.bias is not None else torch.zeros(self.h, **f32))
            self._a1 = torch.zeros(n, self.h, **f32)
            self._wf, self._bf = torch.empty(self.h, self.h, **f32), torch.empty(self.h, **f32)
            check(lib.gd_layer1_fold_f32(ptr(self._w1), ptr(self._b1), ptr(self.wd1), ptr(self._wf), ptr(self._bf), stream_ptr(dev)),
                  'gd_layer1_fold_f32')
            self._cs1 = torch.zeros(max(1, lib.gd_rows_gemm_wgrad_blocks(self.s1)) * self.h, **f32)
            rest = torch.ones(n, dtype=torch.bool, device=dev)
            if self._rows_only:
                rest.zero_()
                rest[self.idx2.long()] = True
            rest[self.idx1.long()] = False
            self._idx1c = rest.nonzero().flatten().to(torch.int32)
            self.pre1.zero_()
        self._chain_expl = plan_explicit_chain(
            self.facts, self.forms,
            self._fold1 and bool(lib.gd_rows_gemm_select_chain_covers(self.s1, int(self._idx1c.numel()), x.shape[1], self.h, self.o)),
            read_explicit_chain(), fold1=self._fold1, n_explicit=int(self._idx1c.numel()) if self._fold1 else 0)
        self._gat_r1 = None
        if self._mode == 'gat':
            w2_ = conv2.lin_src.weight.detach()
            self._gat_r1 = ((conv2.att_src.detach().reshape(1, -1) @ w2_).reshape(-1).float().contiguous(),
                            (conv2.att_dst.detach().reshape(1, -1) @ w2_).reshape(-1).float().contiguous())
        if self._mode == 'rgcn':
            from .graph import TypedNodeCSR
            self.typed = TypedNodeCSR(edge_index, edge_type.to(dev), n, conv2.num_relations)
            self.typed_s1 = None
            if self._rgcn_rows_only and self.s1 > 0:
                in1 = torch.zeros(n, dtype=torch.bool, device=dev)
                in1[self.idx1.long()] = True
                self.typed_s1 = self.typed.restrict_bwd(in1)
            self._hbuf = torch.zeros(n, self.h, **f32)
            self._dxbuf = torch.zeros(n, self.h, **f32)
            for c_, din, dout, tr in ((conv1, self.x.shape[1], self.h, 0), (conv2, self.h, self.o, 0), (conv2, self.o, self.h, 1)):
                if int(lib.gd_rgcn_tile_kl(din, dout, c_.num_blocks or 1, tr)) > 0 and not knobs.rgcn_node_major:
                    tg_ = self.typed_s1 if (tr and self.typed_s1 is not None) else self.typed
                    if ops.rgcn_wave_form(din, dout, c_.num_blocks or 1, n, din) and self.typed.num_relations < 65536:
                        tg_.wave_plan(bool(tr))
                    else:
                        tg_.tile_plan(bool(tr))
                    ops.rgcn_packed_weight(c_.weight.detach(), c_.num_blocks or 1, din, dout, tr)
        if self._mode == 'sage':
            self._w2cat = torch.cat([conv2.lin_l.weight.detach(), conv2.lin_r.weight.detach()], 0).contiguous()
        if self._rows_only:
            from .graph import SplitPlan
            self._plan2 = SplitPlan(self.graph.rowptr, rows=self.idx2)
            self._plan_t1 = SplitPlan(self.graph.rowptr_t, rows=self.idx1)
            self._t1buf = torch.zeros(n, self.h, **f32)
            self._t1rbuf = torch.zeros(n, self.h, **f32) if self._mode == 'sage' else None
            self._t2buf = torch.zeros(n, self.o * (2 if self._mode == 'sage' else 1), **f32)
            self._dt2buf = self._dt2_keep if self._dt2_keep is not None else torch.zeros(n, self.o, **f32)
            self._adots = torch.zeros(2, n, **f32)
            if self._split1:
                self.pre1.zero_()
            self.p2.zero_()
        self.cache_layer1 = cache_layer1
        if cache_layer1:
            with torch.no_grad():
                self._conv1_forward()
                if self._split1:
                    self.p1 = self.pre1
                else:
                    self.p1 = self.z1.clone()
                    if self.s1:
                        self.xs1.copy_(self.p1[self.idx1.long()])

    def _affected_rows_closed(self):
        g, n, dev = self.graph, self.n, self.x.device
        in2 = torch.zeros(n, dtype=torch.bool, device=dev)
        in2[self.idx2.long()] = True
        in1_rows = torch.zeros(n, dtype=torch.bool, device=dev)
        in1_rows[self.idx1.long()] = True
        deg = (g.rowptr[1:] - g.rowptr[:-1]).long()
        erow = torch.repeat_interleave(torch.arange(n, device=dev), deg)
        closed = bool(in2[g.col.long()[in2[erow]]].all()) and bool(in2[self.idx1.long()].all())
        deg_t = (g.rowptr_t[1:] - g.rowptr_t[:-1]).long()
        erow_t = torch.repeat_interleave(torch.arange(n, device=dev), deg_t)
        return closed and bool(in2[g.col_t.long()[in1_rows[erow_t]]].all())

    @staticmethod
    def _mfma_weight(weight):
        out_f, in_f = weight.shape
        return in_f % 32 == 0 and out_f % 32 == 0 and out_f <= 128 and in_f * out_f * 4 <= 64 * 1024

    def _linear(self, x, weight, relu_in=False, idx=None, out=None):
        out_f, in_f = weight.shape
        if idx is not None or self._mfma_weight(weight):
            return ops.rows_gemm(x, idx, weight, trans_w=True, const_w=True, relu_in=relu_in, out=out)
        if ops.mfma_out_width(out_f):
            xin = torch.relu(x) if relu_in else x
            return ops.gemm_wide(xin, ops._const_weight(weight, True)[0], const_x=not relu_in, const_w=True)
        if in_f <= 1024:
            return ops.rows_gemm(x, None, weight, trans_w=True, const_w=True, relu_in=relu_in)
        raise NotImplementedError(f'NodeembEngine: a {in_f} -> {out_f} Linear has no kernel (inputs above 1,024 floats need an output '
                                  'width in {32, 64, 96, 128}); there is no vendor-BLAS fallback')

    def _linear_relu_z1(self, weight, idx=None, out=None):
        if not self._split1:
            return self._linear(self.z1, weight, relu_in=True, idx=idx, out=out)
        if self._chain_expl:
            assert idx is None
            return ops.rows_gemm_select_chain(self._a1, self._idx1c, self._w1, self._b1, self.pre1, self.z1, self.idx1, weight, out=out)
        if idx is not None or self._mfma_weight(weight):
            return ops.rows_gemm_select(self.pre1, self.z1, self._sel1, weight, trans_w=True, const_w=True, relu_in=True,
                                        out=out, idx=idx)
        z = torch.where(self._sel1.bool()[:, None], self.z1, self.pre1)
        return self._linear(z, weight, relu_in=True)

    def _layer1_rows(self, weight):
        if self._rows_only and self._split1 and self._mfma_weight(weight):
            return self.idx2, self._t1buf, self._plan2
        return None, None, None

    def _conv1_forward(self):
        c = self.model.conv1
        g = self.graph
        if self._mode == 'rgcn':
            self._rgcn_conv(c, self.x, self.pre1, 0)
        elif self._mode == 'gcn' and self._fold1:
            self._spmm(False, g.val, self.x, self._a1, None, 0.0, plan=self._plan2 if self._rows_only else None)
            if self._idx1c.numel() and not self._chain_expl:
                ops.rows_gemm(self._a1, self._idx1c, self._w1, trans_w=True, const_w=True, bias=self._b1, out=self.pre1)
        elif self._mode == 'gcn':
            idx, out, plan = self._layer1_rows(c.lin.weight)
            self._spmm(False, g.val, self._linear(self.x, c.lin.weight, idx=idx, out=out), self.pre1, c.bias, 0.0, plan=plan)
        elif self._mode == 'gin':
            lin = c.nn
            if lin.out_features <= lin.in_features:
                idx, out, plan = self._layer1_rows(lin.weight)
                self._spmm(False, None, self._linear(self.x, lin.weight, idx=idx, out=out), self.pre1, lin.bias, 1.0 + c.eps, plan=plan)
            else:
                agg = torch.empty_like(self.x)
                self._spmm(False, None, self.x, agg, None, 1.0 + c.eps)
                ops.rows_gemm(agg, None, lin.weight, trans_w=True, const_w=True, bias=lin.bias, out=self.pre1)
        elif self._mode == 'sage':
            idx, out, plan = self._layer1_rows(c.lin_l.weight)
            t_l = self._linear(self.x, c.lin_l.weight, idx=idx, out=out)
            if (idx is None and self._mfma_weight(c.lin_r.weight)
                    and ops.rows_gemm_accumulate_ok(self.n, c.lin_r.weight.shape[1], c.lin_r.weight.shape[0])
                    and not self.knobs.sage_root_in_spmm):
                self._spmm(False, g.val, t_l, self.pre1, c.lin_l.bias, 0.0)
                ops.rows_gemm_accumulate_(self.pre1, self.x, None, c.lin_r.weight, trans_w=True, const_w=True)
            else:
                t_r = self._linear(self.x, c.lin_r.weight, idx=idx, out=None if idx is None else self._t1rbuf)
                self._spmm(False, g.val, t_l, self.pre1, c.lin_l.bias, 1.0, x_self=t_r, plan=plan)
        else:
            wsrc = c.lin_src.weight
            idx, out, _ = self._layer1_rows(wsrc)
            if idx is None and self._gat_dots and ops.rows_gemm_dots_ok(wsrc.shape[1], wsrc.shape[0], self.n):
                h1, a_src, a_dst = ops.rows_gemm_dots(self.x, wsrc, c.att_src, c.att_dst, const_w=True)
            else:
                h1 = self._linear(self.x, wsrc, idx=idx, out=out)
                a_src, a_dst = ops.row_dots(h1, c.att_src, c.att_dst)
            ops.gat_forward_raw(g, h1, a_src, a_dst, c.bias, c.negative_slope, out=self.pre1,
                                plan=self._plan2 if (self._rows_only and self._split1) else None)

    def _rgcn_conv(self, conv, inp, out, trans, relu_in=False):
        tg = self.typed
        nb = conv.num_blocks or 1
        ops.rows_gemm(inp, None, conv.root.detach(), trans_w=bool(trans), bias=None if trans else conv.bias.detach(), out=out,
                      relu_in=relu_in)
        ops.rgcn_typed_accumulate(tg, inp, conv.weight.detach(), nb, int(trans), out, relu_in=relu_in)

    def _conv2_forward(self):
        c = self.model.conv2
        if self._mode == 'rgcn':
            if self._split1:
                torch.where(self._sel1.bool()[:, None], self.z1, self.pre1, out=self._hbuf)
                self._hbuf.clamp_(min=0)
                self._rgcn_conv(c, self._hbuf, self.p2, 0)
            elif ops.rgcn_wave_relu_ok(self.typed, self.z1, self.p2, c.num_blocks or 1) and not self.knobs.rgcn_relu_pass:
                self._rgcn_conv(c, self.z1, self.p2, 0, relu_in=True)
            else:
                torch.clamp(self.z1, min=0, out=self._hbuf)
                self._rgcn_conv(c, self._hbuf, self.p2, 0)
        elif self._mode in ('gcn', 'gin', 'sage'):
            idx, out, plan = (self.idx2, self._t2buf, self._plan2) if self._rows_only else (None, None, None)
            if self._mode == 'gcn':
                self._spmm(False, self.graph.val, self._linear_relu_z1(c.lin.weight, idx, out), self.p2, c.bias, 0.0, plan=plan)
            elif self._mode == 'gin':
                lin = c.nn
                if lin.out_features > lin.in_features:
                    raise NotImplementedError('GIN layer that widens its input is not on the fused path')
                self._spmm(False, None, self._linear_relu_z1(lin.weight, idx, out), self.p2, lin.bias, 1.0 + c.eps, plan=plan)
            else:
                t2 = self._linear_relu_z1(self._w2cat, idx, out)
                self._spmm(False, self.graph.val, t2[:, :self.o], self.p2, c.lin_l.bias, 1.0, x_self=t2[:, self.o:], plan=plan)
        else:
            wsrc = c.lin_src.weight
            if self._gat_dots and self._split1 and ops.rows_gemm_dots_ok(wsrc.shape[1], wsrc.shape[0], self.s2 if self._rows_only else self.n,
                                                                        selected=self._rows_only):
                ro = self._rows_only
                h2, self._a_src, self._a_dst = ops.rows_gemm_dots(
                    self.pre1, wsrc, c.att_src, c.att_dst, inp_alt=self.z1, sel=self._sel1, relu_in=True, const_w=True,
                    out=self._t2buf if ro else None, idx=self.idx2 if ro else None,
                    dots_out=(self._adots[0], self._adots[1]) if ro else None)
            else:
                h2 = self._linear_relu_z1(wsrc)
                self._a_src, self._a_dst = ops.row_dots(h2, c.att_src, c.att_dst)
            self._h2 = h2
            _, self._rowmax, self._rowsum = ops.gat_forward_raw(self.graph, h2, self._a_src, self._a_dst, c.bias,
                                                                c.negative_slope, out=self.p2,
                                                                plan=self._plan2 if self._rows_only else None)

    def _conv2_backward_to_s1(self):
        c = self.model.conv2
        g = self.graph
        if self._mode == 'rgcn':
            if self.typed_s1 is not None:
                ops.rows_gemm(self.dz2, self.idx1, c.root.detach(), trans_w=True, out=self._dxbuf)
                ops.rgcn_typed_accumulate(self.typed_s1, self.dz2, c.weight.detach(), c.num_blocks or 1, 1, self._dxbuf)
            else:
                self._rgcn_conv(c, self.dz2, self._dxbuf, 1)
            ops.gate_rows(self._dxbuf, self.idx1, self.z1_pos, self.dh)
            return
        if self._mode == 'sage':
            self._spmm(True, g.val_t, self.dz2, self.dcat[:, :self.o], None, 0.0,
                       plan=self._plan_t1 if self._rows_only else None)
            dt2, w2 = self.dcat, self._w2cat
        elif self._mode in ('gcn', 'gin'):
            chain = self._chain1
            if self._rows_only:
                dt2, plan = self._dt2buf, self._plan_t1
            else:
                dt2, plan = (self._dt2_keep if chain else torch.empty(self.n, self.o, dtype=torch.float32, device=self.x.device)), None
            if self._mode == 'gcn':
                self._spmm(True, g.val_t, self.dz2, dt2, None, 0.0, plan=plan)
                w2 = c.lin.weight
            else:
                self._spmm(True, None, self.dz2, dt2, None, 1.0 + c.eps, plan=plan)
                w2 = c.nn.weight
            if chain:
                return
        else:
            chain = self._chain1
            dt2, da_s, da_d = ops.gat_backward_raw(g, self._h2, self._a_src, self._a_dst, self._rowmax, self._rowsum,
                                                   self.dz2, c.negative_slope,
                                                   plan=self._plan2 if self._rows_only else None,
                                                   plan_t=self._plan_t1 if self._rows_only else None,
                                                   bufs=self._gat_bufs if chain else None)
            if chain:
                return
            w2 = c.lin_src.weight
            if self._mfma_weight(w2) and not self.knobs.no_gat_rank1_epilogue:
                ops.rows_gemm(dt2, self.idx1, w2, trans_w=False, out=self.dh, gate_bits=self.z1_pos,
                              rank1=(da_s, self._gat_r1[0], da_d, self._gat_r1[1]))
                return
            ops.rank1_add2_(dt2, da_s, c.att_src, da_d, c.att_dst)
        ops.rows_gemm(dt2, self.idx1, w2, trans_w=False, out=self.dh, gate_bits=self.z1_pos)

    def _spmm(self, transposed, val, x, y, bias, self_coef, x_self=None, plan=None):
        g = self.graph
        if transposed:
            ops._spmm_raw(g.rowptr_t, g.col_t, val, x, bias, self_coef, self.n, plan or g.plan_t, out=y, x_self=x_self)
        else:
            ops._spmm_raw(g.rowptr, g.col, val, x, bias, self_coef, self.n, plan or g.plan, out=y, x_self=x_self)

    def _wgrad(self, a_compact, g, g_idx, n_sel, out, accumulate, ws, adam=None, g_add=None, a_idx=None):
        d_a, d_b = a_compact.shape[1], g.shape[1]
        if adam is not None:
            adam.applied += 1
        if adam is None or self._tail:
            if adam is not None:
                self._tail_acc[0 if adam is self.adam1 else 1] = int(accumulate)
            check(_lib.lib().gd_rows_gemm_wgrad_f32(ptr(a_compact), a_compact.stride(0), ptr(a_idx), ptr(g), g.stride(0),
                                                    ptr(g_idx), None, ptr(g_add), n_sel, d_a, d_b, ptr(out) if adam is None else None,
                                                    int(accumulate), ptr(ws), stream_ptr(g.device)),
                  'gd_rows_gemm_wgrad_f32')
            return
        check(_lib.lib().gd_rows_gemm_wgrad_adam_f32(
            ptr(a_compact), a_compact.stride(0), ptr(a_idx), ptr(g), g.stride(0), ptr(g_idx), None, ptr(g_add), n_sel,
            d_a, d_b, ptr(out), int(accumulate), ptr(ws), ptr(adam.param), ptr(adam.m), ptr(adam.v),
            ptr(adam.iter_ctr), adam.lr, adam.betas[0], adam.betas[1], adam.eps, stream_ptr(g.device)),
            'gd_rows_gemm_wgrad_adam_f32')

    def _wgrad1(self, accumulate, g_add):
        assert not self._fold1, 'the folded layer-1 step never forms pre1 on the Del-1 rows: its weight gradient comes out of the chained pass'
        a1, a1_idx = (self.pre1, self.idx1) if self._split1 else (self.xs1, None)
        if not self._fuse_loss1:
            self._wgrad(a1, self.dz1, self.idx1, self.s1, self.g1, accumulate, self.ws1, adam=self.adam1,
                        g_add=g_add, a_idx=a1_idx)
            return
        a = self.adam1
        a.applied += 1
        if self._tail:
            self._tail_acc[0] = int(accumulate)
        check(_lib.lib().gd_rows_gemm_wgrad_loss_f32(
            ptr(a1), a1.stride(0), ptr(a1_idx), ptr(self.z1), self.z1.stride(0), ptr(self.idx1),
            ptr(self._slot1), ptr(self.t1.tm), ptr(self.t1.coef), ptr(self._cnt_signed1), ptr(g_add), self.s1, self.h,
            self.h, None if self._tail else ptr(self.g1), int(accumulate), ptr(self.ws1), ptr(self._lp1),
            None if self._tail else ptr(a.param), ptr(a.m), ptr(a.v),
            ptr(a.iter_ctr), a.lr, a.betas[0], a.betas[1], a.eps, stream_ptr(self.x.device)),
            'gd_rows_gemm_wgrad_loss_f32')

    def _iteration(self):
        lt = self.loss_type
        with torch.no_grad(), ops.keep_constants(self._const_refs):
            if not self.cache_layer1:
                self._conv1_forward()
            if self.cache_layer1 and not self._split1:
                ops.rows_gemm(self.p1, self.idx1, self.wd1, out=self.z1, sign_bits=self.z1_pos)
            elif self._fuse_del1:
                self._del1_fused(self.dh if lt == 'both_layerwise' else None)
            else:
                assert not self._fold1
                ops.rows_gemm(self.pre1, self.idx1, self.wd1, out=self.z1, save_in=self.xs1, sign_bits=self.z1_pos)
            fused_fin = self.t1.folded and self.t2.folded
            if not fused_fin:
                self.sums.zero_()
            s1 = None if fused_fin else self.sums[0:2]
            s2 = None if fused_fin else self.sums[2:4]
            if not self._fuse_loss1 and lt != 'only2_all':
                self.t1.launch(self.z1, self.dz1, s1)
            elif self._out1 and lt != 'only2_all' and not self._out_pair:
                self.t1.launch_outside(self.z1, None, self._lp1[2 * self._lp1_blocks:])
            if self._fuse_del1:
                pass
            elif lt == 'both_layerwise':
                self._wgrad1(False, self.dh)
            elif lt == 'only1':
                self._wgrad1(False, None)
            self._conv2_forward()
            if self._fuse_l2:
                self._del2_fused()
                if self._out2 and self._out_pair and lt != 'only2_all':
                    check(_lib.lib().gd_rowtarget_mse_pair_f32(
                        *self.t1.outside_args(self.z1, None, self._lp1[2 * self._lp1_blocks:]),
                        *self.t2.outside_args(self.p2, self.dz2, self._lp2[2 * self._lp2_blocks:]), stream_ptr(self.x.device)),
                        'gd_rowtarget_mse_pair_f32')
                elif self._out2:
                    self.t2.launch_outside(self.p2, self.dz2, self._lp2[2 * self._lp2_blocks:])
            else:
                ops.rows_gemm(self.p2, self.idx2, self.wd2, out=self.z2, save_in=self.xs2)
                self.t2.launch(self.z2, self.dz2, s2)
            if lt == 'both_layerwise':
                self._layer2_backward()
            elif lt == 'both_all':
                self._layer2_backward(g2_accumulate=True)
                self._wgrad1(True, self.dh)
            elif lt == 'only2_layerwise':
                self._layer2_backward(to_w1=False)
            elif lt == 'only2_all':
                self._layer2_backward()
                a1, a1_idx = (self.pre1, self.idx1) if self._split1 else (self.xs1, None)
                self._wgrad(a1, self.dh, self.idx1, self.s1, self.g1, False, self.ws1, adam=self.adam1, a_idx=a1_idx)
            if lt != 'only1' and not self._fuse_l2 and not self._tail:
                self.adam2.apply(self.g2)
            p1, n1 = ((self._lp1, self._lp1_blocks + (self.t1.outside_blocks() if self._out1 else 0)) if self._fuse_loss1
                      else (self.t1.partials, self.t1.n_partial_blocks()))
            p2, n2 = ((self._lp2, self._lp2_blocks + (self.t2.outside_blocks() if self._out2 else 0)) if self._fuse_l2
                      else (self.t2.partials, self.t2.n_partial_blocks()))
            if self._tail:
                a1, a2 = self.adam1, self.adam2
                lib_ = _lib.lib()
                nw1 = self._lp1_blocks if self._fuse_del1 else lib_.gd_rows_gemm_wgrad_blocks(self.s1)
                if self._fold1:
                    check(lib_.gd_step_tail_fold1_f32(
                        ptr(self.ws1), ptr(self._cs1), nw1, self.h, self._tail_acc[0], ptr(self._w1), ptr(self._b1), ptr(self.g1),
                        ptr(a1.param), ptr(a1.m), ptr(a1.v), ptr(self._wf), ptr(self._bf),
                        ptr(self.ws2), self._lp2_blocks if self._fuse_wg2 else lib_.gd_rows_gemm_wgrad_blocks(self.s2), self.o,
                        self._tail_acc[1], ptr(self.g2), ptr(a2.param), ptr(a2.m), ptr(a2.v), a1.lr, a1.betas[0], a1.betas[1], a1.eps,
                        ptr(p1), n1, ptr(p2), n2, ptr(self.hist), self.hist.shape[0], ptr(self.hist_pos), ptr(self.iter_ctr),
                        ptr(self._arrive), stream_ptr(self.x.device)), 'gd_step_tail_fold1_f32')
                else:
                    check(lib_.gd_step_tail_parts_f32(
                        ptr(self.ws1), nw1, self.h, self._tail_acc[0], ptr(self.g1), ptr(a1.param), ptr(a1.m), ptr(a1.v),
                        ptr(self.ws2), self._lp2_blocks if self._fuse_wg2 else lib_.gd_rows_gemm_wgrad_blocks(self.s2), self.o,
                        self._tail_acc[1], ptr(self.g2), ptr(a2.param),
                        ptr(a2.m), ptr(a2.v), a1.lr, a1.betas[0], a1.betas[1], a1.eps, ptr(p1), n1, ptr(p2), n2, ptr(self.hist),
                        self.hist.shape[0], ptr(self.hist_pos), ptr(self.iter_ctr), ptr(self._arrive), stream_ptr(self.x.device)),
                        'gd_step_tail_parts_f32')
            else:
                check(_lib.lib().gd_loss_finalize_f32(
                    ptr(p1) if fused_fin else None, n1 if fused_fin else 0,
                    ptr(p2) if fused_fin else None, n2 if fused_fin else 0,
                    None if fused_fin else ptr(self.sums), ptr(self.hist), self.hist.shape[0], ptr(self.hist_pos),
                    ptr(self.iter_ctr), stream_ptr(self.x.device)), 'gd_loss_finalize_f32')
            if self._user_wd2 is not None:
                self._user_wd2.data.copy_(self.wd2.data[:self._o_true, :self._o_true])

    def _conv2_weight(self):
        c2 = self.model.conv2
        return (c2.lin if self._mode == 'gcn' else c2.nn).weight.detach()

    def _del1_fused(self, g_add):
        self.adam1.applied += 1
        self._tail_acc[0] = 0
        if self._chain1:
            c2 = self.model.conv2
            if self._mode == 'gat':
                w_next, dt = c2.lin_src.weight.detach(), self._gat_bufs['dh']
                rank1 = (ptr(self._gat_bufs['da_src']), ptr(self._gat_r1[0]), ptr(self._gat_bufs['da_dst']), ptr(self._gat_r1[1]))
            else:
                w_next, dt = self._conv2_weight(), self._dt2_keep
                if self._fold2:
                    w_next = self._w2fold
                rank1 = (None, None, None, None)
            if self._fold1:
                check(_lib.lib().gd_del1_chain_fold_loss_wgrad_f32(
                    ptr(self._a1), self._a1.stride(0), ptr(self.idx1), self.s1, ptr(self._wf), ptr(self._bf), self.h, ptr(self.z1),
                    self.z1.stride(0), ptr(self.z1_pos), ptr(self._slot1), ptr(self.t1.tm), ptr(self.t1.coef), ptr(self._cnt_signed1),
                    ptr(dt), dt.stride(0), self.o, ptr(w_next), ptr(self._lp1), ptr(self.ws1), ptr(self._cs1), self._lp1_blocks,
                    stream_ptr(self.x.device)), 'gd_del1_chain_fold_loss_wgrad_f32')
                return
            check(_lib.lib().gd_del1_chain_loss_wgrad_f32(
                ptr(self.pre1), self.pre1.stride(0), ptr(self.idx1), self.s1, ptr(self.wd1), self.h, ptr(self.z1), self.z1.stride(0),
                ptr(self.z1_pos), ptr(self._slot1), ptr(self.t1.tm), ptr(self.t1.coef), ptr(self._cnt_signed1), ptr(dt),
                dt.stride(0), self.o, ptr(w_next), *rank1, ptr(self._lp1), ptr(self.ws1), self._lp1_blocks,
                stream_ptr(self.x.device)), 'gd_del1_chain_loss_wgrad_f32')
            return
        check(_lib.lib().gd_del1_loss_wgrad_f32(
            ptr(self.pre1), self.pre1.stride(0), ptr(self.idx1), self.s1, ptr(self.wd1), self.h, ptr(self.z1), self.z1.stride(0),
            ptr(self.z1_pos), ptr(self._slot1), ptr(self.t1.tm), ptr(self.t1.coef), ptr(self._cnt_signed1), ptr(g_add),
            g_add.stride(0) if g_add is not None else 0, ptr(self._lp1), ptr(self.ws1), self._lp1_blocks, stream_ptr(self.x.device)),
            'gd_del1_loss_wgrad_f32')

    def _del2_fused(self):
        if self._fold2:
            w2 = self._conv2_weight()
            check(_lib.lib().gd_del_loss_fold_wgrad_parts_f32(
                ptr(self.p2), self.p2.stride(0), ptr(self.idx2), self.s2, ptr(self.wd2), self.o, ptr(self._slot2),
                ptr(self.t2.tm), ptr(self.t2.coef), ptr(self._cnt_signed2), ptr(self.dz2), self.dz2.stride(0), ptr(w2), self.h,
                ptr(self._w2fold), ptr(self._lp2), ptr(self.ws2), self._lp2_blocks, stream_ptr(self.x.device)),
                'gd_del_loss_fold_wgrad_parts_f32')
            return
        if self._fuse_wg2:
            check(_lib.lib().gd_del_loss_bwd_wgrad_parts_f32(
                ptr(self.p2), self.p2.stride(0), ptr(self.idx2), self.s2, ptr(self.wd2), self.o, ptr(self._slot2),
                ptr(self.t2.tm), ptr(self.t2.coef), ptr(self._cnt_signed2), None, self.o,
                ptr(self.dz2), self.dz2.stride(0), ptr(self._lp2), ptr(self.ws2), self._lp2_blocks, stream_ptr(self.x.device)),
                'gd_del_loss_bwd_wgrad_parts_f32')
            return
        check(_lib.lib().gd_del_loss_bwd_f32(
            ptr(self.p2), self.p2.stride(0), ptr(self.idx2), self.s2, ptr(self.wd2), self.o, ptr(self._slot2),
            ptr(self.t2.tm), ptr(self.t2.coef), ptr(self._cnt_signed2), ptr(self.dz2c), self.dz2c.stride(0),
# ... 95 lines not shown
```

### gnndelete_amd/ops.py

```python
import os

import torch

from . import _lib
from ._lib import check, ptr, stream_ptr


def matrix_split():
    return _lib.lib().gd_matrix_split()


def set_matrix_split(n_products):
    _lib.check(_lib.lib().gd_set_matrix_split(int(n_products)), 'gd_set_matrix_split')


def _f32_rows(t):
    if t.device.type != 'cuda':
        raise _lib.GnnDeleteHipError('gnndelete_amd ops need CUDA(HIP) tensors; got a CPU tensor (no CPU fallback)')
    if t.dtype != torch.float32:
        t = t.float()
    if t.dim() != 2 or t.stride(1) != 1 or t.stride(0) < t.shape[1] or (t.stride(0) % 4 and t.shape[1] % 4 == 0):
        t = t.contiguous()
    return t




def _spmm_raw(rowptr, col, val, x, bias, self_coef, n_rows, plan=None, out=None, x_self=None, wide=True):
    d = x.shape[1]
    if x_self is not None:
        assert plan is not None and x_self.stride(0) == x.stride(0) and x_self.shape[1] == d
    y = out if out is not None else torch.empty(n_rows, d, dtype=torch.float32, device=x.device)
    if (plan is not None and d % 4 == 0 and d <= 1024 and x.stride(0) % 4 == 0 and x.data_ptr() % 16 == 0
            and os.environ.get('GD_SPMM_TWO_LAUNCH') != '1'):
        x_rows = max(int(x.shape[0]), int(y.shape[0]))
        if (wide and d == 64 and x_rows < (1 << 24) and x.stride(0) * 4 < (1 << 24) and y.stride(0) * 4 < (1 << 24)
                and x_rows * x.stride(0) * 4 < (1 << 32) and x_rows * y.stride(0) * 4 < (1 << 32)
                and os.environ.get('GD_SPMM_MULTIROW') != '0' and not os.environ.get('GD_SPMM_D64_FORM')):
            items, n_items, bounds, tags = plan.onepass_wide(d)
            check(_lib.lib().gd_spmm_csr_onepass_wide_f32(ptr(items), n_items, ptr(_wide_col(plan, col, tags)), ptr(val), ptr(x), x.stride(0),
                                                          ptr(y), y.stride(0), ptr(bias), float(self_coef), ptr(x_self), d,
                                                          int(col.shape[0]), x_rows, ptr(bounds), stream_ptr(x.device)),
                  'gd_spmm_csr_onepass_wide_f32')
            return y
        items, n_items, bounds = plan.onepass(d)
        check(_lib.lib().gd_spmm_csr_onepass_f32(ptr(items), n_items, ptr(col), ptr(val), ptr(x), x.stride(0), ptr(y),
                                                 y.stride(0), ptr(bias), float(self_coef), ptr(x_self), d, int(col.shape[0]),
                                                 max(int(x.shape[0]), int(y.shape[0])), ptr(bounds), stream_ptr(x.device)),
              'gd_spmm_csr_onepass_f32')
        return y
    if plan is not None and d % 4 == 0 and d <= 1024 and x.stride(0) % 4 == 0 and x.data_ptr() % 16 == 0:
        scratch = plan.scratch(d, x.device)
        check(_lib.lib().gd_spmm_csr_balanced_f32(ptr(plan.items), plan.n_items, ptr(plan.split), plan.n_split,
                                                  ptr(col), ptr(val), ptr(x), x.stride(0), ptr(y), y.stride(0),
                                                  ptr(bias), float(self_coef), ptr(x_self), ptr(scratch), d, int(col.shape[0]),
                                                  max(int(x.shape[0]), int(y.shape[0])), ptr(plan.xcd_bounds(d)),
                                                  stream_ptr(x.device)),
              'gd_spmm_csr_balanced_f32')
        return y
    assert x_self is None, 'x_self needs the balanced kernel (d % 4 == 0, 16-byte aligned rows)'
    check(_lib.lib().gd_spmm_csr_f32(ptr(rowptr), ptr(col), ptr(val), ptr(x), x.stride(0), ptr(y), y.stride(0),
                                     ptr(bias), float(self_coef), n_rows, d, stream_ptr(x.device)),
          'gd_spmm_csr_f32')
    return y


class _SpMM(torch.autograd.Function):

    @staticmethod
    def forward(ctx, x, bias, graph, self_coef):
        x = _f32_rows(x)
        ctx.graph, ctx.self_coef = graph, self_coef
        ctx.has_bias = bias is not None
        return _spmm_raw(graph.rowptr, graph.col, graph.val, x, bias, self_coef, graph.n, graph.plan)

    @staticmethod
    def backward(ctx, dy):
        g = ctx.graph
        dx = db = None
        if ctx.needs_input_grad[0]:
            dx = _spmm_raw(g.rowptr_t, g.col_t, g.val_t, _f32_rows(dy), None, ctx.self_coef, g.n, g.plan_t)
        if ctx.has_bias and ctx.needs_input_grad[1]:
            db = dy.sum(0)
        return dx, db, None, None


def spmm(x, graph, bias=None, self_coef=0.0):
    return _SpMM.apply(x, bias, graph, self_coef)


_SINKS = []


class keep_constants:

    def __init__(self, store):
        self.store = store

    def __enter__(self):
        _SINKS.append(self.store)
        return self.store

    def __exit__(self, *exc):
        _SINKS.pop()


def _note_constant(t):
    for store in _SINKS:
        store[id(t)] = t
    return t


def _lru_get(cache, key, capacity, build):
    hit = cache.pop(key, None)
    if hit is None:
        while len(cache) >= capacity:
            cache.pop(next(iter(cache)))
        hit = build()
    cache[key] = hit
    return hit


def _wide_col(plan, col, tags):
    def build():
        assert tags.shape[0] == col.shape[0], 'the plan was built for another CSR'
        return (col | (tags << 24)).contiguous(), col, tags
    hit = _lru_get(plan._wide_cols, (col.data_ptr(), int(col.shape[0]), col._version, tags.data_ptr()), 4, build)
    return _note_constant(hit[0])


_WT_CACHE = {}


# ... 856 lines not shown
```

### include/gnndelete_hip.h

```cpp
#ifndef GNNDELETE_HIP_H
#define GNNDELETE_HIP_H

#include <stdint.h>

#ifdef __cplusplus
extern "C" {
#endif

#define GD_ABI_VERSION 9

enum {
  GD_OK = 0,
  GD_E_NULL = 1,
  GD_E_DIM = 2,
  GD_E_ALIGN = 3,
  GD_E_WORKSPACE = 4
};

int gd_abi_version(void);
const char* gd_last_error_string(void);
const char* gd_build_source_hash(void);

#define GD_MATRIX_SPLIT_DEFAULT 0
int gd_matrix_split(void);
// ... 166 lines not shown
                           const float* g, int64_t ld_g, const int32_t* g_idx,
                           const float* relu_mask, const float* g_add, int32_t n_sel, int32_t d_a,
                           int32_t d_b, float* dw, int32_t accumulate, float* partials, void* stream);

int gd_rows_gemm_wgrad_adam_f32(const float* a, int64_t ld_a, const int32_t* a_idx,
                                const float* g, int64_t ld_g, const int32_t* g_idx,
                                const float* relu_mask, const float* g_add, int32_t n_sel, int32_t d_a,
                                int32_t d_b, float* dw, int32_t accumulate, float* partials,
                                float* param, float* exp_avg, float* exp_avg_sq, const int32_t* iter,
                                double lr, double beta1, double beta2, double eps, void* stream);

int gd_rows_gemm_wgrad_reduce_f32(const float* partials, int32_t n_sel, int32_t d_a, int32_t d_b, float* dw,
                                  int32_t accumulate, float* param, float* exp_avg, float* exp_avg_sq,
                                  const int32_t* iter, double lr, double beta1, double beta2, double eps, void* stream);

int gd_step_tail_f32(const float* partials1, int32_t n_sel1, int32_t d1, int32_t accumulate1, float* dw1, float* param1,
                     float* exp_avg1, float* exp_avg_sq1, const float* partials2, int32_t n_sel2, int32_t d2,
                     int32_t accumulate2, float* dw2, float* param2, float* exp_avg2, float* exp_avg_sq2, double lr,
                     double beta1, double beta2, double eps, const float* loss_partials1, int32_t n1,
                     const float* loss_partials2, int32_t n2, float* hist, int32_t capacity, int32_t* pos, int32_t* iter,
                     int32_t* arrive, void* stream);
int gd_step_tail_parts_f32(const float* partials1, int32_t n_part1, int32_t d1, int32_t accumulate1, float* dw1, float* param1,
                           float* exp_avg1, float* exp_avg_sq1, const float* partials2, int32_t n_part2, int32_t d2,
                           int32_t accumulate2, float* dw2, float* param2, float* exp_avg2, float* exp_avg_sq2, double lr,
                           double beta1, double beta2, double eps, const float* loss_partials1, int32_t n1,
                           const float* loss_partials2, int32_t n2, float* hist, int32_t capacity, int32_t* pos, int32_t* iter,
                           int32_t* arrive, void* stream);

int32_t gd_rows_gemm_wgrad_blocks(int32_t n_sel);
int gd_rows_gemm_wgrad_loss_f32(const float* a, int64_t ld_a, const int32_t* a_idx,
                                const float* z, int64_t ld_z, const int32_t* z_idx,
                                const int32_t* loss_slot, const float* tm, const float* coef,
                                const float* cnt_signed, const float* g_add,
                                int32_t n_sel, int32_t d_a, int32_t d_b, float* dw, int32_t accumulate,
                                float* partials, float* loss_partials,
                                float* param, float* exp_avg, float* exp_avg_sq, const int32_t* iter,
                                double lr, double beta1, double beta2, double eps, void* stream);

int32_t gd_del_loss_bwd_blocks(int32_t n_sel);
int gd_del_loss_bwd_f32(const float* p, int64_t ld_p, const int32_t* idx, int32_t n_sel, const float* w, int32_t d,
                        const int32_t* loss_slot, const float* tm, const float* coef, const float* cnt_signed,
                        float* dz, int64_t ld_dz, float* dp, int64_t ld_dp, float* loss_partials, void* stream);

int gd_del_loss_bwd_wgrad_f32(const float* p, int64_t ld_p, const int32_t* idx, int32_t n_sel, const float* w, int32_t d,
                              const int32_t* loss_slot, const float* tm, const float* coef, const float* cnt_signed,
                              float* dz, int64_t ld_dz, float* dp, int64_t ld_dp, float* loss_partials,
                              float* wgrad_partials, void* stream);
int32_t gd_del_loss_bwd_wgrad_parts(int32_t n_sel, int32_t d);
int gd_del_loss_bwd_wgrad_parts_f32(const float* p, int64_t ld_p, const int32_t* idx, int32_t n_sel, const float* w, int32_t d,
                                    const int32_t* loss_slot, const float* tm, const float* coef, const float* cnt_signed,
                                    float* dz, int64_t ld_dz, float* dp, int64_t ld_dp, float* loss_partials,
                                    float* wgrad_partials, int32_t n_part, void* stream);
int32_t gd_del_loss_fold_wgrad_covers(int32_t n_sel, int32_t d, int32_t h);
int gd_del_loss_fold_wgrad_parts_f32(const float* p, int64_t ld_p, const int32_t* idx, int32_t n_sel, const float* w, int32_t d,
                                     const int32_t* loss_slot, const float* tm, const float* coef, const float* cnt_signed,
                                     float* g, int64_t ld_g, const float* w_next, int32_t h, float* w_fold,
                                     float* loss_partials, float* wgrad_partials, int32_t n_part, void* stream);

int32_t gd_del1_loss_wgrad_covers(int32_t n_sel, int32_t d);
int32_t gd_del1_loss_wgrad_parts(int32_t n_sel);
int gd_del1_loss_wgrad_f32(const float* p, int64_t ld_p, const int32_t* idx, int32_t n_sel, const float* w, int32_t d, float* z,
                           int64_t ld_z, uint32_t* sign_out, const int32_t* loss_slot, const float* tm, const float* coef,
                           const float* cnt_signed, const float* g_add, int64_t ld_gadd, float* loss_partials,
                           float* wgrad_partials, int32_t n_part, void* stream);
int gd_del1_chain_loss_wgrad_f32(const float* p, int64_t ld_p, const int32_t* idx, int32_t n_sel, const float* w, int32_t d, float* z,
                                 int64_t ld_z, uint32_t* sign_io, const int32_t* loss_slot, const float* tm, const float* coef,
                                 const float* cnt_signed, const float* dt, int64_t ld_dt, int32_t d_next, const float* w_next,
                                 const float* row_a, const float* col_a, const float* row_b, const float* col_b,
                                 float* loss_partials, float* wgrad_partials, int32_t n_part, void* stream);

int32_t gd_del1_chain_fold_covers(int32_t n_sel, int32_t d, int32_t h);
int gd_del1_chain_fold_loss_wgrad_f32(const float* a, int64_t ld_a, const int32_t* idx, int32_t n_sel, const float* w_fold,
                                      const float* bias_fold, int32_t d, float* z, int64_t ld_z, uint32_t* sign_io,
                                      const int32_t* loss_slot, const float* tm, const float* coef, const float* cnt_signed,
                                      const float* dt, int64_t ld_dt, int32_t d_next, const float* w_next, float* loss_partials,
                                      float* wgrad_partials_t, float* colsum_partials, int32_t n_part, void* stream);
int gd_layer1_fold_f32(const float* w1, const float* b1, const float* wd, float* w_fold, float* bias_fold, void* stream);
int gd_step_tail_fold1_f32(const float* partials1_t, const float* colsum1, int32_t n_part1, int32_t d1, int32_t accumulate1,
                           const float* w1, const float* b1, float* dw1, float* param1, float* exp_avg1, float* exp_avg_sq1,
                           float* w_fold, float* bias_fold, const float* partials2, int32_t n_part2, int32_t d2, int32_t accumulate2,
                           float* dw2, float* param2, float* exp_avg2, float* exp_avg_sq2, double lr, double beta1, double beta2,
                           double eps, const float* loss_partials1, int32_t n1, const float* loss_partials2, int32_t n2,
                           float* hist, int32_t capacity, int32_t* pos, int32_t* iter, int32_t* arrive, void* stream);


int64_t gd_rowpair_mse_workspace(int32_t n_seg);
int gd_rowpair_mse_f32(const float* z, int64_t ld_z, const float* o, int64_t ld_o, int32_t d,
                       const int32_t* seg_ptr, const int32_t* seg_row, int32_t n_seg,
                       const int32_t* term_o, const float* term_w, const int32_t* term_kind,
                       float* dz, int64_t ld_dz, int32_t dz_compact,
                       float* sums, float* partials, void* stream);

int64_t gd_rowtarget_mse_workspace(int32_t n_rows);
int gd_rowtarget_mse_f32(const float* z, int64_t ld_z, const float* tm, int32_t d,
                         const int32_t* row_idx, const float* coef, const float* cnt, const int32_t* kind,
                         int32_t n_rows, float* dz, int64_t ld_dz, float* sums, float* partials, void* stream);
int32_t gd_rowtarget_mse_pair_covers(int32_t d_a, int32_t d_b);
int gd_rowtarget_mse_pair_f32(const float* z_a, int64_t ld_z_a, const float* tm_a, int32_t d_a, const int32_t* row_idx_a,
                              const float* coef_a, const float* cnt_a, const int32_t* kind_a, int32_t n_rows_a, float* dz_a,
                              int64_t ld_dz_a, float* partials_a, const float* z_b, int64_t ld_z_b, const float* tm_b, int32_t d_b,
                              const int32_t* row_idx_b, const float* coef_b, const float* cnt_b, const int32_t* kind_b,
                              int32_t n_rows_b, float* dz_b, int64_t ld_dz_b, float* partials_b, void* stream);

int32_t gd_rowtarget_mse_blocks(int32_t n_rows);
int gd_loss_finalize_f32(const float* partials1, int32_t n1, const float* partials2, int32_t n2,
                         const float* extra_sums, float* hist, int32_t capacity, int32_t* pos, int32_t* iter,
                         void* stream);

int32_t gd_rowfold_loss_blocks(int32_t n_rows);
int gd_rowfold_loss_f32(int32_t family, const float* z, int64_t ld_z, const float* tm, int32_t d, int32_t d_valid,
                        const int32_t* row_idx, const float* coef, const float* cnt, const int32_t* kind, int32_t n_rows,
                        float* dz, int64_t ld_dz, float* partials, void* stream);
int gd_rowfold_kld_scale_f32(const float* partials, int32_t n_blocks, float k_dec, float k_ni, float inv_n_dec, float inv_n_ni,
                             const int32_t* row_idx, const int32_t* kind, int32_t n_rows, int32_t d, float* dz, int64_t ld_dz,
                             float* scales, void* stream);

int64_t gd_gemm_f32_workspace(int32_t n_rows, int32_t k, int32_t n);
int gd_gemm_f32(const float* in, int64_t ld_in, const int32_t* idx, int32_t n_rows, const float* w, int32_t k,
                int32_t n, const float* bias, float* out, int64_t ld_out, float* workspace, void* stream);

int gd_edge_dot_f32(const float* z, int64_t ld_z, int32_t d, const int64_t* e0, const int64_t* e1,
                    const float* rel, int64_t ld_rel, const int64_t* etype,
                    int64_t n_edges, float* out, void* stream);

int gd_edge_dot_bwd_f32(const float* z, int64_t ld_z, int32_t d, const int32_t* other, const float* w,
                        const float* rel, int64_t ld_rel, const int32_t* etype, const int64_t* inc_ptr,
                        int64_t n_nodes, float* dz, int64_t ld_dz, void* stream);

int64_t gd_pairs_sigmoid_mse_workspace(int32_t n_s, int32_t d);
int gd_pairs_sigmoid_mse_f32(const float* z, int64_t ld_z, const int32_t* nodes, int32_t n_s, int32_t d,
                             const float* target, int64_t ld_t, float inv_count,
                             float* loss, float* dz, float* workspace, void* stream);


int64_t gd_edgeprob_dec_workspace(int64_t m, int32_t d);
int gd_edgeprob_dec_f32(const float* z, int64_t ld_z, int64_t n_nodes, int32_t d, const int64_t* pos, int64_t ld_pos,
                        const int64_t* neg, int64_t ld_neg, int64_t m, float coef, float* w, float* loss,
                        const int32_t* src_edge, const int64_t* inc_ptr, float* w_inc, float* workspace, void* stream);

int64_t gd_edge_incidence_workspace(int64_t n_nodes, int64_t n_edges);
int gd_edge_incidence(const int64_t* e0, const int64_t* e1, int64_t n_edges, int64_t n_nodes, int64_t* inc_ptr,
                      int32_t* other, int32_t* src_edge, void* workspace, int64_t workspace_bytes, void* stream);

int64_t gd_edge_incidence_fixed_bytes(int64_t n_nodes, int64_t n_fixed);
int gd_edge_incidence_fixed(const int64_t* e0, const int64_t* e1, int64_t n_fixed, int64_t n_nodes, void* image, int64_t image_bytes,
                            void* workspace, int64_t workspace_bytes, void* stream);
int64_t gd_edge_incidence_update_workspace(int64_t n_nodes, int64_t n_edges);
int gd_edge_incidence_update(const void* image, const int64_t* e0, const int64_t* e1, int64_t n_fixed, int64_t n_edges,
                             int64_t n_nodes, int64_t* inc_ptr, int32_t* other, int32_t* src_edge, void* workspace,
                             int64_t workspace_bytes, void* stream);

int gd_rows_add_f32(float* dz, int64_t ld_dz, int64_t n_rows, const int32_t* nodes, int32_t n_s, const float* src,
                    int64_t ld_src, float scale, int32_t d, void* stream);

int gd_edgeprob_record_f32(const float* loss_r, const float* loss_l, float coef_r, float coef_l, float* hist,
                           int32_t capacity, int32_t* pos, void* stream);

int64_t gd_edgeprob_batch_loss_workspace(int64_t k, int64_t n_cand, int32_t d);
int gd_edgeprob_batch_loss_f32(const float* z, int64_t ld_z, int64_t n_nodes, const float* z_ori, int64_t ld_ori, int64_t n_ori,
                               int32_t d, const int64_t* pos, int64_t ld_pos, const int64_t* neg, int64_t ld_neg, int64_t k,
                               const int64_t* cand_src, const int64_t* cand_dst, int64_t n_cand, float coef_e, float coef_l,
                               int64_t* dec, int64_t ld_dec, float* w, float* losses, int64_t* inc_ptr, int32_t* other,
                               int32_t* src_edge, float* w_inc, void* inc_workspace, int64_t inc_workspace_bytes,
                               float* workspace, void* stream);


// ... 84 lines not shown
```

Measured before the change: 2140 iters/s.

## Run step-tail Adam/fold jobs as extra blocks inside the wide SpMM launch

Adds a hosted variant of the wide 64-float SpMM kernel whose first blocks run the step-tail work (weight-gradient partial reduction, Adam updates, layer-1 fold, loss finalize), while the remaining blocks do the aggregation. The tail code moves into a shared header so both kernels can use it. The goal is to remove the separate tail kernel launch and overlap the small tail work with the bandwidth-bound SpMM. The cost is more complex cross-block dependencies through the arrive/iter counters, and the tail blocks may compete with SpMM blocks for CUs.

```diff
diff --git a/gnndelete_amd/_lib.py b/gnndelete_amd/_lib.py
--- a/gnndelete_amd/_lib.py
+++ b/gnndelete_amd/_lib.py
@@ -112,6 +112,10 @@
     'gd_layer1_fold_f32': (ctypes.c_int, [_p, _p, _p, _p, _p, _p]),
     'gd_step_tail_fold1_f32': (ctypes.c_int, [_p, _p, _i32, _i32, _i32, _p, _p, _p, _p, _p, _p, _p, _p, _p, _i32, _i32, _i32, _p, _p, _p, _p,
                                               _f64, _f64, _f64, _f64, _p, _i32, _p, _i32, _p, _i32, _p, _p, _p, _p]),
+    'gd_spmm_csr_onepass_wide_hosted_f32': (ctypes.c_int, [_p, _i32, _p, _p, _p, _i64, _p, _i64, _p, _f32, _p, _i32, _i32, _i32, _p,
+                                                           _p, _p, _i32, _i32, _p, _p, _p, _p, _p, _p, _p, _p, _p,
+                                                           _p, _i32, _i32, _i32, _p, _p, _p, _p, _f64, _f64, _f64, _f64,
+                                                           _p, _i32, _p, _i32, _p, _i32, _p, _p, _p, _p]),
     'gd_del1_loss_wgrad_f32': (ctypes.c_int, [_p, _i64, _p, _i32, _p, _i32, _p, _i64, _p, _p, _p, _p, _p, _p, _i64, _p, _p, _i32, _p]),
     'gd_rowtarget_mse_blocks': (_i32, [_i32]),
     'gd_rowfold_loss_blocks': (_i32, [_i32]),
diff --git a/gnndelete_amd/csrc/rows_gemm.hip b/gnndelete_amd/csrc/rows_gemm.hip
--- a/gnndelete_amd/csrc/rows_gemm.hip
+++ b/gnndelete_amd/csrc/rows_gemm.hip
@@ -1,4 +1,5 @@
 #include "common.h"
+#include "tail_jobs.h"
 
 namespace gd {
 
@@ -664,85 +665,6 @@
   }
 }
 
-struct TailJob {
-  const float* partials; int32_t n_part, n_elem, accumulate;
-  float* dw; float* param; float* m; float* v;
-};
-struct TailFin {
-  const float* p1; int32_t n1; const float* p2; int32_t n2;
-  float* hist; int32_t capacity; int32_t* pos; int32_t* iter; int32_t* arrive;
-};
-
-__device__ __forceinline__ int32_t tail_check_in(const TailFin& fin) {
-  int32_t t = atomicAdd(fin.iter, 0);
-  asm volatile("" : "+v"(t));
-  atomicAdd(fin.arrive + (t < 0 ? 1 : 0), 1);
-  return t + 1;
-}
-
-__device__ __forceinline__ void tail_job_block(const TailJob& j, int blk, const TailFin& fin, float4 (*red)[16], int32_t* t_sh, double lr,
-                                               double beta1, double beta2, double eps) {
-  const int tid = threadIdx.x;
-  if (tid == 0) *t_sh = tail_check_in(fin);
-  const int vv = tid & 15, slice = tid >> 4;
-  const int e4 = blk * 16 + vv;
-  const int n4 = j.n_elem >> 2;
-  float4 s0 = f4_zero(), s1 = f4_zero(), s2 = f4_zero(), s3 = f4_zero();
-  if (e4 < n4) {
-    int b = slice;
-    for (; b + 48 < j.n_part; b += 64) {
-      const float4 p0 = reinterpret_cast<const float4*>(j.partials + (int64_t)b * j.n_elem)[e4];
-      const float4 p1 = reinterpret_cast<const float4*>(j.partials + (int64_t)(b + 16) * j.n_elem)[e4];
-      const float4 p2 = reinterpret_cast<const float4*>(j.partials + (int64_t)(b + 32) * j.n_elem)[e4];
-      const float4 p3 = reinterpret_cast<const float4*>(j.partials + (int64_t)(b + 48) * j.n_elem)[e4];
-      s0 = f4_add(s0, p0); s1 = f4_add(s1, p1); s2 = f4_add(s2, p2); s3 = f4_add(s3, p3);
-    }
-    for (; b < j.n_part; b += 16) s0 = f4_add(s0, reinterpret_cast<const float4*>(j.partials + (int64_t)b * j.n_elem)[e4]);
-  }
-  red[slice][vv] = f4_add(f4_add(s0, s1), f4_add(s2, s3));
-  __syncthreads();
-  if (slice == 0 && e4 < n4) {
-    float4 t4 = j.accumulate ? reinterpret_cast<float4*>(j.dw)[e4] : f4_zero();
-#pragma unroll
-    for (int i = 0; i < 16; ++i) t4 = f4_add(t4, red[i][vv]);
-    reinterpret_cast<float4*>(j.dw)[e4] = t4;
-    const AdamScalars sc = adam_scalars(lr, beta1, beta2, eps, *t_sh);
-    float4 p4 = reinterpret_cast<float4*>(j.param)[e4], m4 = reinterpret_cast<float4*>(j.m)[e4],
-           v4 = reinterpret_cast<float4*>(j.v)[e4];
-    adam_update(p4.x, m4.x, v4.x, t4.x, sc);
-    adam_update(p4.y, m4.y, v4.y, t4.y, sc);
-    adam_update(p4.z, m4.z, v4.z, t4.z, sc);
-    adam_update(p4.w, m4.w, v4.w, t4.w, sc);
-    reinterpret_cast<float4*>(j.param)[e4] = p4;
-    reinterpret_cast<float4*>(j.m)[e4] = m4;
-    reinterpret_cast<float4*>(j.v)[e4] = v4;
-  }
-}
-
-__device__ __forceinline__ void tail_finalize_block(const TailFin& fin, float (*fred)[256], int n_wait) {
-  const int tid = threadIdx.x;
-  float a = 0.f, b = 0.f, c = 0.f, d = 0.f;
-  for (int i = tid; i < fin.n1; i += 256) { a += fin.p1[2 * i]; b += fin.p1[2 * i + 1]; }
-  for (int i = tid; i < fin.n2; i += 256) { c += fin.p2[2 * i]; d += fin.p2[2 * i + 1]; }
-  fred[0][tid] = a; fred[1][tid] = b; fred[2][tid] = c; fred[3][tid] = d;
-  __syncthreads();
-  for (int off = 128; off > 0; off >>= 1) {
-    if (tid < off) {
-#pragma unroll
-      for (int q = 0; q < 4; ++q) fred[q][tid] += fred[q][tid + off];
-    }
-    __syncthreads();
-  }
-  if (tid < 4) fin.hist[(int64_t)(*fin.pos) * 4 + tid] = fred[tid][0];
-  __syncthreads();
-  if (tid == 0) {
-    while (atomicAdd(fin.arrive, 0) < n_wait) __builtin_amdgcn_s_sleep(8);
-    *fin.arrive = 0;
-    *fin.pos = (*fin.pos + 1) % fin.capacity;
-    atomicAdd(fin.iter, 1);
-  }
-}
-
 __global__ __launch_bounds__(256) void step_tail_kernel(TailJob j1, TailJob j2, TailFin fin, double lr, double beta1, double beta2,
                                                         double eps) {
   __shared__ float4 red[16][16];
@@ -755,39 +677,6 @@
     return;
   }
   tail_finalize_block(fin, fred, nb1 + nb2);
-}
-
-__device__ __forceinline__ void fold1_column(const float* w1s, const float* __restrict__ b1, const float* wd_col, int c, float* scr,
-                                             float* __restrict__ wf, float* __restrict__ bf) {
-  const int tid = threadIdx.x, i = tid & 127, hf = tid >> 7;
-  float acc = 0.f;
-#pragma unroll 16
-  for (int j = 64 * hf; j < 64 * hf + 64; ++j) acc = fmaf(w1s[j * 129 + i], wd_col[j], acc);
-  scr[tid] = acc;
-  __syncthreads();
-  if (tid < 128) wf[(int64_t)tid * 128 + c] = scr[tid] + scr[tid + 128];
-  __syncthreads();
-  scr[tid] = tid < 128 ? b1[tid] * wd_col[tid] : 0.f;
-  __syncthreads();
-  for (int off = 64; off > 0; off >>= 1) {
-    if (tid < off) scr[tid] += scr[tid + off];
-    __syncthreads();
-  }
-  if (tid == 0) bf[c] = scr[0];
-  __syncthreads();
-}
-
-__device__ __forceinline__ void fold1_fetch_w1(const float* __restrict__ w1, float4 (&r)[16]) {
-#pragma unroll
-  for (int it = 0; it < 16; ++it) r[it] = reinterpret_cast<const float4*>(w1)[threadIdx.x + 256 * it];
-}
-__device__ __forceinline__ void fold1_store_w1(const float4 (&r)[16], float* w1s) {
-#pragma unroll
-  for (int it = 0; it < 16; ++it) {
-    const int e = threadIdx.x + 256 * it;
-    float* dst = w1s + (e >> 5) * 129 + (e & 31) * 4;
-    dst[0] = r[it].x; dst[1] = r[it].y; dst[2] = r[it].z; dst[3] = r[it].w;
-  }
 }
 
 __global__ __launch_bounds__(256) void layer1_fold_kernel(const float* __restrict__ w1, const float* __restrict__ b1, const float* __restrict__ wd,
@@ -801,10 +690,8 @@
   if (threadIdx.x < 128) wd_col[threadIdx.x] = wd[(int64_t)threadIdx.x * 128 + c];
   fold1_store_w1(w1r, w1s);
   __syncthreads();
-  fold1_column(w1s, b1, wd_col, c, scr, wf, bf);
-}
-
-struct TailFold1 { const float* colsum; const float* w1; const float* b1; float* wf; float* bf; };
+  fold1_column<129>(w1s, b1, wd_col, c, scr, wf, bf);
+}
 
 __global__ __launch_bounds__(256) void step_tail_fold1_kernel(TailJob j1, TailJob j2, TailFin fin, TailFold1 fo, double lr, double beta1,
                                                               double beta2, double eps) {
@@ -815,67 +702,10 @@
   __shared__ int32_t t_sh;
   constexpr int D = 128;
   const int nb2 = (j2.n_elem / 4 + 15) / 16;
-  const int tid = threadIdx.x;
   if ((int)blockIdx.x >= D + nb2) { tail_finalize_block(fin, fred, D + nb2); return; }
   if ((int)blockIdx.x >= D) { tail_job_block(j2, blockIdx.x - D, fin, red, &t_sh, lr, beta1, beta2, eps); return; }
-  const int c = blockIdx.x;
-  if (tid == 0) t_sh = tail_check_in(fin);
-  float4 w1r[16];
-  fold1_fetch_w1(fo.w1, w1r);
-  {
-    const int vv = tid & 31, slice = tid >> 5;
-    const float4* src = reinterpret_cast<const float4*>(j1.partials + (int64_t)c * D) + vv;
-    const int64_t pitch4 = (int64_t)D * D / 4;
-    float4 sa[8];
-#pragma unroll
-    for (int q = 0; q < 8; ++q) sa[q] = f4_zero();
-    int b = slice;
-    for (; b + 56 < j1.n_part; b += 64) {
-      float4 pv[8];
-#pragma unroll
-      for (int q = 0; q < 8; ++q) pv[q] = src[(b + 8 * q) * pitch4];
-#pragma unroll
-      for (int q = 0; q < 8; ++q) sa[q] = f4_add(sa[q], pv[q]);
-    }
-    for (; b < j1.n_part; b += 8) sa[0] = f4_add(sa[0], src[b * pitch4]);
-    float4* const red8 = &red[0][0];
-    red8[slice * 32 + vv] = f4_add(f4_add(f4_add(sa[0], sa[1]), f4_add(sa[2], sa[3])), f4_add(f4_add(sa[4], sa[5]), f4_add(sa[6], sa[7])));
-    float cs = 0.f;
-    for (int q = tid; q < j1.n_part; q += 256) cs += fo.colsum[(int64_t)q * D + c];
-    fred[0][tid] = cs;
-    fold1_store_w1(w1r, w1s);
-    __syncthreads();
-    if (tid < 32) {
-      float4 t4 = red8[tid];
-#pragma unroll
-      for (int i = 1; i < 8; ++i) t4 = f4_add(t4, red8[i * 32 + tid]);
-      reinterpret_cast<float4*>(gcol)[tid] = t4;
-    }
-    for (int off = 128; off > 0; off >>= 1) {
-      if (tid < off) fred[0][tid] += fred[0][tid + off];
-      __syncthreads();
-    }
-  }
-  {
-    const int j = tid & 127, hf = tid >> 7;
-    float acc = 0.f;
-#pragma unroll 16
-    for (int i = 64 * hf; i < 64 * hf + 64; ++i) acc = fmaf(w1s[j * 129 + i], gcol[i], acc);
-    fred[1][tid] = acc;
-    __syncthreads();
-    if (tid < D) {
-      const float g = fmaf(fo.b1[tid], fred[0][0], fred[1][tid] + fred[1][tid + 128]);
-      const int64_t e = (int64_t)tid * D + c;
-      j1.dw[e] = g;
-      const AdamScalars sc = adam_scalars(lr, beta1, beta2, eps, t_sh);
-      float pv = j1.param[e], mv = j1.m[e], vv = j1.v[e];
-      adam_update(pv, mv, vv, g, sc);
-      j1.param[e] = pv; j1.m[e] = mv; j1.v[e] = vv;
-      wd_col[tid] = pv;
-    }
-    __syncthreads();
-  }
-  fold1_column(w1s, fo.b1, wd_col, c, fred[2], fo.wf, fo.bf);
+  if (threadIdx.x == 0) t_sh = tail_check_in(fin);
+  tail_fold1_column_block<true>(j1, fo, nullptr, blockIdx.x, w1s, &red[0][0], fred, gcol, wd_col, &t_sh, lr, beta1, beta2, eps);
 }
 
 __global__ __launch_bounds__(256) void wgrad_reduce_scalar_kernel(const float* __restrict__ partials, int32_t n_part,
diff --git a/gnndelete_amd/csrc/spmm.hip b/gnndelete_amd/csrc/spmm.hip
--- a/gnndelete_amd/csrc/spmm.hip
+++ b/gnndelete_amd/csrc/spmm.hip
@@ -2,6 +2,7 @@
 #include <string.h>
 
 #include "common.h"
+#include "tail_jobs.h"
 
 namespace gd {
 
@@ -360,17 +361,17 @@
 #define GD_SPMM_WIDE_GRID_CAP 8192
 #endif
 
-__global__ __launch_bounds__(256) __attribute__((amdgpu_waves_per_eu(8, 8))) void spmm_wide_kernel(
+__device__ __forceinline__ void spmm_wide_body(
     const int4* __restrict__ items, int32_t n_items, const int32_t* __restrict__ xcd_bounds, const int32_t* __restrict__ colt,
     const float* __restrict__ val, const float* __restrict__ x, int64_t ldx, float* __restrict__ y, int64_t ldy,
-    const float* __restrict__ bias, float self_coef, const float* __restrict__ xs, int32_t nnz) {
+    const float* __restrict__ bias, float self_coef, const float* __restrict__ xs, int32_t nnz, uint32_t bid, uint32_t nblk) {
   constexpr int kXcd = 8, U = 4;
   constexpr int kSrcMask = (1 << 24) - 1;
   const int lane = threadIdx.x & 63;
   const int g = lane >> 4, li = lane & 15;
-  const int xcd = blockIdx.x % kXcd;
-  const int stride = (gridDim.x / kXcd) * 4;
-  const int wx = (blockIdx.x / kXcd) * 4 + (threadIdx.x >> 6);
+  const int xcd = bid % kXcd;
+  const int stride = (nblk / kXcd) * 4;
+  const int wx = (bid / kXcd) * 4 + (threadIdx.x >> 6);
   const int i0 = xcd_bounds[xcd], i1 = xcd_bounds[xcd + 1];
   if ((i0 | i1) & 3) __builtin_trap();
   const uint32_t lo = 16u * (uint32_t)li;
@@ -530,6 +531,24 @@
   }
 }
 
+__global__ __launch_bounds__(256) __attribute__((amdgpu_waves_per_eu(8, 8))) void spmm_wide_kernel(
+    const int4* __restrict__ items, int32_t n_items, const int32_t* __restrict__ xcd_bounds, const int32_t* __restrict__ colt,
+    const float* __restrict__ val, const float* __restrict__ x, int64_t ldx, float* __restrict__ y, int64_t ldy,
+    const float* __restrict__ bias, float self_coef, const float* __restrict__ xs, int32_t nnz) {
+  spmm_wide_body(items, n_items, xcd_bounds, colt, val, x, ldx, y, ldy, bias, self_coef, xs, nnz, blockIdx.x, gridDim.x);
+}
+
+__global__ __launch_bounds__(256) __attribute__((amdgpu_waves_per_eu(8, 8))) void spmm_wide_hosted_kernel(
+    const int4* __restrict__ items, int32_t n_items, const int32_t* __restrict__ xcd_bounds, const int32_t* __restrict__ colt,
+    const float* __restrict__ val, const float* __restrict__ x, int64_t ldx, float* __restrict__ y, int64_t ldy,
+    const float* __restrict__ bias, float self_coef, const float* __restrict__ xs, int32_t nnz, TailHost host) {
+  if (blockIdx.x < (uint32_t)host.nh) {
+    tail_host_block(host, (int)blockIdx.x);
+    return;
+  }
+  spmm_wide_body(items, n_items, xcd_bounds, colt, val, x, ldx, y, ldy, bias, self_coef, xs, nnz, blockIdx.x - host.nh, gridDim.x - host.nh);
+}
+
 __global__ __launch_bounds__(256) void spmm_fixup_kernel(const int4* __restrict__ split, int32_t n_split,
                                                          const float* __restrict__ scratch,
                                                          const float* __restrict__ x, int64_t ldx,
@@ -766,32 +785,86 @@
                         xcd_bounds, (hipStream_t)stream);
 }
 
-extern "C" int gd_spmm_csr_onepass_wide_f32(const int32_t* items, int32_t n_items, const int32_t* col_tagged, const float* val,
-                                            const float* x, int64_t ldx, float* y, int64_t ldy, const float* bias,
-                                            float self_coef, const float* x_self, int32_t d, int32_t nnz, int32_t x_rows,
-                                            const int32_t* xcd_bounds, void* stream) {
-  using namespace gd;
-  GD_REQUIRE(col_tagged && x && y && xcd_bounds && (items || n_items == 0), GD_E_NULL, "gd_spmm_csr_onepass_wide_f32: null pointer");
+namespace gd {
+static int launch_wide(const char* name, const int32_t* items, int32_t n_items, const int32_t* col_tagged, const float* val, const float* x,
+                       int64_t ldx, float* y, int64_t ldy, const float* bias, float self_coef, const float* x_self, int32_t d,
+                       int32_t nnz, int32_t x_rows, const int32_t* xcd_bounds, const TailHost* host, void* stream) {
+  GD_REQUIRE(col_tagged && x && y && xcd_bounds && (items || n_items == 0), GD_E_NULL, "%s: null pointer", name);
   GD_REQUIRE(n_items >= 0 && n_items % 4 == 0 && d == 64 && ldx % 4 == 0 && ldy % 4 == 0 && ldx >= d && ldy >= d, GD_E_DIM,
-             "gd_spmm_csr_onepass_wide_f32: d must be 64 (got %d) with 16-byte row strides, n_items a multiple of 4", d);
-  GD_REQUIRE(aligned16(x) && aligned16(y) && aligned16(items) && (!bias || aligned16(bias)), GD_E_ALIGN,
-             "gd_spmm_csr_onepass_wide_f32: unaligned pointer");
-  GD_REQUIRE(x != y, GD_E_DIM, "gd_spmm_csr_onepass_wide_f32: x and y must not alias");
+             "%s: d must be 64 (got %d) with 16-byte row strides, n_items a multiple of 4", name, d);
+  GD_REQUIRE(aligned16(x) && aligned16(y) && aligned16(items) && (!bias || aligned16(bias)), GD_E_ALIGN, "%s: unaligned pointer", name);
+  GD_REQUIRE(x != y, GD_E_DIM, "%s: x and y must not alias", name);
   GD_REQUIRE(x_rows > 0 && x_rows < (1 << 24) && ldx * 4 < (1 << 24) && ldy * 4 < (1 << 24) &&
                  (int64_t)x_rows * ldx * 4 < (1ll << 32) && (int64_t)x_rows * ldy * 4 < (1ll << 32), GD_E_DIM,
-             "gd_spmm_csr_onepass_wide_f32: x and y must be smaller than 4 GiB with row ids and pitches below 2^24");
+             "%s: x and y must be smaller than 4 GiB with row ids and pitches below 2^24", name);
+  GD_REQUIRE(!host || n_items > 0, GD_E_DIM, "%s: the tail's jobs need a launch to ride on (n_items = 0)", name);
   if (n_items == 0) return GD_OK;
   const float* xs = x_self ? x_self : x;
-  GD_REQUIRE(aligned16(xs) && xs != y, GD_E_ALIGN, "gd_spmm_csr_onepass_wide_f32: bad x_self");
+  GD_REQUIRE(aligned16(xs) && xs != y, GD_E_ALIGN, "%s: bad x_self", name);
   const char* e = getenv("GD_SPMM_GRID_CAP");
   const int cap_env = e ? atoi(e) : 0;
   const int cap = cap_env > 0 ? cap_env : GD_SPMM_WIDE_GRID_CAP;
   int nblk = (n_items + 3) / 4;
   if (nblk > cap) nblk = cap;
   nblk = (nblk + 7) / 8 * 8;
+  if (host) {
+    hipLaunchKernelGGL(spmm_wide_hosted_kernel, dim3(host->nh + nblk), dim3(256), 0, (hipStream_t)stream,
+                       reinterpret_cast<const int4*>(items), n_items, xcd_bounds, col_tagged, val, x, ldx, y, ldy, bias, self_coef, xs, nnz,
+                       *host);
+    return launched("spmm_wide_hosted");
+  }
   hipLaunchKernelGGL(spmm_wide_kernel, dim3(nblk), dim3(256), 0, (hipStream_t)stream, reinterpret_cast<const int4*>(items), n_items,
                      xcd_bounds, col_tagged, val, x, ldx, y, ldy, bias, self_coef, xs, nnz);
   return launched("spmm_wide");
+}
+}
+
+extern "C" int gd_spmm_csr_onepass_wide_f32(const int32_t* items, int32_t n_items, const int32_t* col_tagged, const float* val,
+                                            const float* x, int64_t ldx, float* y, int64_t ldy, const float* bias,
+                                            float self_coef, const float* x_self, int32_t d, int32_t nnz, int32_t x_rows,
+                                            const int32_t* xcd_bounds, void* stream) {
+  return gd::launch_wide("gd_spmm_csr_onepass_wide_f32", items, n_items, col_tagged, val, x, ldx, y, ldy, bias, self_coef, x_self, d, nnz,
+                         x_rows, xcd_bounds, nullptr, stream);
+}
+
+extern "C" int gd_spmm_csr_onepass_wide_hosted_f32(
+    const int32_t* items, int32_t n_items, const int32_t* col_tagged, const float* val, const float* x, int64_t ldx, float* y, int64_t ldy,
+    const float* bias, float self_coef, const float* x_self, int32_t d, int32_t nnz, int32_t x_rows, const int32_t* xcd_bounds,
+    const float* partials1_t, const float* colsum1, int32_t n_part1, int32_t d1, const float* w1, const float* w1_t, const float* b1,
+    float* dw1, float* param1, float* exp_avg1, float* exp_avg_sq1, float* w_fold, float* bias_fold, const float* partials2,
+    int32_t n_part2, int32_t d2, int32_t accumulate2, float* dw2, float* param2, float* exp_avg2, float* exp_avg_sq2, double lr,
+    double beta1, double beta2, double eps, const float* loss_partials1, int32_t n1, const float* loss_partials2, int32_t n2, float* hist,
+    int32_t capacity, int32_t* pos, int32_t* iter, int32_t* arrive, void* stream) {
+  using namespace gd;
+  const char* name = "gd_spmm_csr_onepass_wide_hosted_f32";
+  GD_REQUIRE(n_part1 >= 0 && n_part2 >= 0 && n_part1 + n_part2 > 0, GD_E_DIM,
+             "%s: a hosted launch carries job 1, job 2 or both (partial counts %d, %d)", name, n_part1, n_part2);
+  GD_REQUIRE(iter, GD_E_NULL, "%s: null iteration counter", name);
+  TailHost h{};
+  h.lr = lr; h.beta1 = beta1; h.beta2 = beta2; h.eps = eps;
+  h.fin = TailFin{loss_partials1, n1, loss_partials2, n2, hist, capacity, pos, iter, arrive};
+  if (n_part1 > 0) {
+    GD_REQUIRE(partials1_t && colsum1 && w1 && w1_t && b1 && dw1 && param1 && exp_avg1 && exp_avg_sq1 && w_fold && bias_fold, GD_E_NULL,
+               "%s: null pointer of job 1", name);
+    GD_REQUIRE(d1 == 128, GD_E_DIM, "%s: the folded layer-1 job is 128 wide (d1=%d)", name, d1);
+    GD_REQUIRE(aligned16(partials1_t), GD_E_ALIGN, "%s: unaligned partials of job 1", name);
+    h.j1 = TailJob{partials1_t, n_part1, d1 * d1, 0, dw1, param1, exp_avg1, exp_avg_sq1};
+    h.fo = TailFold1{colsum1, w1, b1, w_fold, bias_fold};
+    h.w1t = w1_t;
+    h.n1b = 128;
+  }
+  if (n_part2 > 0) {
+    GD_REQUIRE(partials2 && dw2 && param2 && exp_avg2 && exp_avg_sq2, GD_E_NULL, "%s: null pointer of job 2", name);
+    GD_REQUIRE(hist && pos && arrive && capacity > 0 && n1 >= 0 && n2 >= 0 && (n1 == 0 || loss_partials1) && (n2 == 0 || loss_partials2),
+               GD_E_NULL, "%s: null bookkeeping pointer", name);
+    GD_REQUIRE(d2 > 0 && d2 % 4 == 0 && d2 <= 128, GD_E_DIM, "%s: d2=%d must be a multiple of 4, at most 128", name, d2);
+    GD_REQUIRE(aligned16(partials2) && aligned16(dw2) && aligned16(param2) && aligned16(exp_avg2) && aligned16(exp_avg_sq2), GD_E_ALIGN,
+               "%s: unaligned pointer of job 2", name);
+    h.j2 = TailJob{partials2, n_part2, d2 * d2, accumulate2, dw2, param2, exp_avg2, exp_avg_sq2};
+    h.nb2 = (h.j2.n_elem / 4 + 15) / 16;
+  }
+  h.nh = (h.n1b + h.nb2 + 7) / 8 * 8;
+  return launch_wide(name, items, n_items, col_tagged, val, x, ldx, y, ldy, bias, self_coef, x_self, d, nnz, x_rows, xcd_bounds, &h, stream);
 }
 
 extern "C" int gd_spmm_csr_onepass_aux_f32(const int32_t* items, int32_t n_items, const int32_t* col, const int32_t* perm,
diff --git a/gnndelete_amd/csrc/tail_jobs.h b/gnndelete_amd/csrc/tail_jobs.h
--- /dev/null
+++ b/gnndelete_amd/csrc/tail_jobs.h
@@ -0,0 +1,236 @@
+#pragma once
+#include "common.h"
+
+namespace gd {
+
+struct TailJob {
+  const float* partials; int32_t n_part, n_elem, accumulate;
+  float* dw; float* param; float* m; float* v;
+};
+struct TailFin {
+  const float* p1; int32_t n1; const float* p2; int32_t n2;
+  float* hist; int32_t capacity; int32_t* pos; int32_t* iter; int32_t* arrive;
+};
+struct TailFold1 { const float* colsum; const float* w1; const float* b1; float* wf; float* bf; };
+
+__device__ __forceinline__ int32_t tail_check_in(const TailFin& fin) {
+  int32_t t = atomicAdd(fin.iter, 0);
+  asm volatile("" : "+v"(t));
+  atomicAdd(fin.arrive + (t < 0 ? 1 : 0), 1);
+  return t + 1;
+}
+
+__device__ __forceinline__ void tail_reduce_adam(const TailJob& j, int blk, float4 (*red)[16], const int32_t* t_sh, double lr, double beta1,
+                                                 double beta2, double eps) {
+  const int tid = threadIdx.x;
+  const int vv = tid & 15, slice = tid >> 4;
+  const int e4 = blk * 16 + vv;
+  const int n4 = j.n_elem >> 2;
+  float4 s0 = f4_zero(), s1 = f4_zero(), s2 = f4_zero(), s3 = f4_zero();
+  if (e4 < n4) {
+    int b = slice;
+    for (; b + 48 < j.n_part; b += 64) {
+      const float4 p0 = reinterpret_cast<const float4*>(j.partials + (int64_t)b * j.n_elem)[e4];
+      const float4 p1 = reinterpret_cast<const float4*>(j.partials + (int64_t)(b + 16) * j.n_elem)[e4];
+      const float4 p2 = reinterpret_cast<const float4*>(j.partials + (int64_t)(b + 32) * j.n_elem)[e4];
+      const float4 p3 = reinterpret_cast<const float4*>(j.partials + (int64_t)(b + 48) * j.n_elem)[e4];
+      s0 = f4_add(s0, p0); s1 = f4_add(s1, p1); s2 = f4_add(s2, p2); s3 = f4_add(s3, p3);
+    }
+    for (; b < j.n_part; b += 16) s0 = f4_add(s0, reinterpret_cast<const float4*>(j.partials + (int64_t)b * j.n_elem)[e4]);
+  }
+  red[slice][vv] = f4_add(f4_add(s0, s1), f4_add(s2, s3));
+  __syncthreads();
+  if (slice == 0 && e4 < n4) {
+    float4 t4 = j.accumulate ? reinterpret_cast<float4*>(j.dw)[e4] : f4_zero();
+#pragma unroll
+    for (int i = 0; i < 16; ++i) t4 = f4_add(t4, red[i][vv]);
+    reinterpret_cast<float4*>(j.dw)[e4] = t4;
+    const AdamScalars sc = adam_scalars(lr, beta1, beta2, eps, *t_sh);
+    float4 p4 = reinterpret_cast<float4*>(j.param)[e4], m4 = reinterpret_cast<float4*>(j.m)[e4],
+           v4 = reinterpret_cast<float4*>(j.v)[e4];
+    adam_update(p4.x, m4.x, v4.x, t4.x, sc);
+    adam_update(p4.y, m4.y, v4.y, t4.y, sc);
+    adam_update(p4.z, m4.z, v4.z, t4.z, sc);
+    adam_update(p4.w, m4.w, v4.w, t4.w, sc);
+    reinterpret_cast<float4*>(j.param)[e4] = p4;
+    reinterpret_cast<float4*>(j.m)[e4] = m4;
+    reinterpret_cast<float4*>(j.v)[e4] = v4;
+  }
+}
+
+__device__ __forceinline__ void tail_job_block(const TailJob& j, int blk, const TailFin& fin, float4 (*red)[16], int32_t* t_sh, double lr,
+                                               double beta1, double beta2, double eps) {
+  if (threadIdx.x == 0) *t_sh = tail_check_in(fin);
+  tail_reduce_adam(j, blk, red, t_sh, lr, beta1, beta2, eps);
+}
+
+__device__ __forceinline__ void tail_finalize_sums(const TailFin& fin, float (*fred)[256]) {
+  const int tid = threadIdx.x;
+  float a = 0.f, b = 0.f, c = 0.f, d = 0.f;
+  for (int i = tid; i < fin.n1; i += 256) { a += fin.p1[2 * i]; b += fin.p1[2 * i + 1]; }
+  for (int i = tid; i < fin.n2; i += 256) { c += fin.p2[2 * i]; d += fin.p2[2 * i + 1]; }
+  fred[0][tid] = a; fred[1][tid] = b; fred[2][tid] = c; fred[3][tid] = d;
+  __syncthreads();
+  for (int off = 128; off > 0; off >>= 1) {
+    if (tid < off) {
+#pragma unroll
+      for (int q = 0; q < 4; ++q) fred[q][tid] += fred[q][tid + off];
+    }
+    __syncthreads();
+  }
+  if (tid < 4) fin.hist[(int64_t)(*fin.pos) * 4 + tid] = fred[tid][0];
+  __syncthreads();
+}
+
+__device__ __forceinline__ void tail_finalize_block(const TailFin& fin, float (*fred)[256], int n_wait) {
+  tail_finalize_sums(fin, fred);
+  if (threadIdx.x == 0) {
+    while (atomicAdd(fin.arrive, 0) < n_wait) __builtin_amdgcn_s_sleep(8);
+    *fin.arrive = 0;
+    *fin.pos = (*fin.pos + 1) % fin.capacity;
+    atomicAdd(fin.iter, 1);
+  }
+}
+
+template <int SK>
+__device__ __forceinline__ float tail_chain64(const float* mat, const float* vec, int k0) {
+  float acc = 0.f;
+#pragma unroll 16
+  for (int k = k0; k < k0 + 64; ++k) acc = fmaf(mat[k * SK], vec[k], acc);
+  return acc;
+}
+
+template <int LD>
+__device__ __forceinline__ void fold1_column(const float* w1m, const float* __restrict__ b1, const float* wd_col, int c, float* scr,
+                                             float* __restrict__ wf, float* __restrict__ bf) {
+  const int tid = threadIdx.x, i = tid & 127, hf = tid >> 7;
+  scr[tid] = tail_chain64<LD>(w1m + i, wd_col, 64 * hf);
+  __syncthreads();
+  if (tid < 128) wf[(int64_t)tid * 128 + c] = scr[tid] + scr[tid + 128];
+  __syncthreads();
+  scr[tid] = tid < 128 ? b1[tid] * wd_col[tid] : 0.f;
+  __syncthreads();
+  for (int off = 64; off > 0; off >>= 1) {
+    if (tid < off) scr[tid] += scr[tid + off];
+    __syncthreads();
+  }
+  if (tid == 0) bf[c] = scr[0];
+  __syncthreads();
+}
+
+__device__ __forceinline__ void fold1_fetch_w1(const float* __restrict__ w1, float4 (&r)[16]) {
+#pragma unroll
+  for (int it = 0; it < 16; ++it) r[it] = reinterpret_cast<const float4*>(w1)[threadIdx.x + 256 * it];
+}
+__device__ __forceinline__ void fold1_store_w1(const float4 (&r)[16], float* w1s) {
+#pragma unroll
+  for (int it = 0; it < 16; ++it) {
+    const int e = threadIdx.x + 256 * it;
+    float* dst = w1s + (e >> 5) * 129 + (e & 31) * 4;
+    dst[0] = r[it].x; dst[1] = r[it].y; dst[2] = r[it].z; dst[3] = r[it].w;
+  }
+}
+
+template <bool IMAGE>
+__device__ __forceinline__ void tail_fold1_column_block(const TailJob& j1, const TailFold1& fo, const float* __restrict__ w1t, int c,
+                                                        float* w1s, float4* red8, float (*fred)[256], float* gcol, float* wd_col,
+                                                        const int32_t* t_sh, double lr, double beta1, double beta2, double eps) {
+  constexpr int D = 128;
+  constexpr int F = IMAGE ? 8 : 4;
+  const int tid = threadIdx.x;
+  float4 w1r[IMAGE ? 16 : 1];
+  if constexpr (IMAGE) fold1_fetch_w1(fo.w1, w1r);
+  {
+    const int vv = tid & 31, slice = tid >> 5;
+    const float4* src = reinterpret_cast<const float4*>(j1.partials + (int64_t)c * D) + vv;
+    const int64_t pitch4 = (int64_t)D * D / 4;
+    float4 sa[8];
+#pragma unroll
+    for (int q = 0; q < 8; ++q) sa[q] = f4_zero();
+    int b = slice;
+    for (; b + 56 < j1.n_part; b += 64) {
+#pragma unroll
+      for (int q0 = 0; q0 < 8; q0 += F) {
+        float4 pv[F];
+#pragma unroll
+        for (int q = 0; q < F; ++q) pv[q] = src[(b + 8 * (q0 + q)) * pitch4];
+#pragma unroll
+        for (int q = 0; q < F; ++q) sa[q0 + q] = f4_add(sa[q0 + q], pv[q]);
+        if constexpr (!IMAGE) __builtin_amdgcn_sched_barrier(0);
+      }
+    }
+    for (; b < j1.n_part; b += 8) sa[0] = f4_add(sa[0], src[b * pitch4]);
+    red8[slice * 32 + vv] = f4_add(f4_add(f4_add(sa[0], sa[1]), f4_add(sa[2], sa[3])), f4_add(f4_add(sa[4], sa[5]), f4_add(sa[6], sa[7])));
+    float cs = 0.f;
+    for (int q = tid; q < j1.n_part; q += 256) cs += fo.colsum[(int64_t)q * D + c];
+    fred[0][tid] = cs;
+    if constexpr (IMAGE) fold1_store_w1(w1r, w1s);
+    __syncthreads();
+    if (tid < 32) {
+      float4 t4 = red8[tid];
+#pragma unroll
+      for (int i = 1; i < 8; ++i) t4 = f4_add(t4, red8[i * 32 + tid]);
+      reinterpret_cast<float4*>(gcol)[tid] = t4;
+    }
+    for (int off = 128; off > 0; off >>= 1) {
+      if (tid < off) fred[0][tid] += fred[0][tid + off];
+      __syncthreads();
+    }
+  }
+  {
+    const int j = tid & 127, hf = tid >> 7;
+    fred[1][tid] = IMAGE ? tail_chain64<1>(w1s + j * 129, gcol, 64 * hf) : tail_chain64<D>(w1t + j, gcol, 64 * hf);
+    __syncthreads();
+    if (tid < D) {
+      const float g = fmaf(fo.b1[tid], fred[0][0], fred[1][tid] + fred[1][tid + 128]);
+      const int64_t e = (int64_t)tid * D + c;
+      j1.dw[e] = g;
+      const AdamScalars sc = adam_scalars(lr, beta1, beta2, eps, *t_sh);
+      float pv = j1.param[e], mv = j1.m[e], vv = j1.v[e];
+      adam_update(pv, mv, vv, g, sc);
+      j1.param[e] = pv; j1.m[e] = mv; j1.v[e] = vv;
+      wd_col[tid] = pv;
+    }
+    __syncthreads();
+  }
+  if constexpr (IMAGE) fold1_column<129>(w1s, fo.b1, wd_col, c, fred[2], fo.wf, fo.bf);
+  else fold1_column<D>(fo.w1, fo.b1, wd_col, c, fred[2], fo.wf, fo.bf);
+}
+
+struct TailHost {
+  TailJob j1, j2; TailFin fin; TailFold1 fo; const float* w1t;
+  int32_t n1b, nb2, nh;
+  double lr, beta1, beta2, eps;
+};
+
+__device__ __forceinline__ void tail_host_block(const TailHost& h, int blk) {
+  __shared__ float4 red[16][16];
+  __shared__ float fred[4][256];
+  __shared__ float gcol[128], wd_col[128];
+  __shared__ int32_t t_sh, last_sh;
+  const int tid = threadIdx.x;
+  if (blk >= h.n1b + h.nb2) return;
+  if (tid == 0) t_sh = atomicAdd(h.fin.iter, 0) + 1;
+  if (blk < h.n1b) {
+    tail_fold1_column_block<false>(h.j1, h.fo, h.w1t, blk, nullptr, &red[0][0], fred, gcol, wd_col, &t_sh, h.lr, h.beta1, h.beta2, h.eps);
+    if (h.nb2 == 0) return;
+  } else {
+    tail_reduce_adam(h.j2, blk - h.n1b, red, &t_sh, h.lr, h.beta1, h.beta2, h.eps);
+  }
+  __syncthreads();
+  if (tid == 0) {
+    int32_t t = t_sh;
+    asm volatile("" : "+v"(t));
+    last_sh = atomicAdd(h.fin.arrive + (t < 1 ? 1 : 0), 1) == h.n1b + h.nb2 - 1;
+  }
+  __syncthreads();
+  if (!last_sh) return;
+  tail_finalize_sums(h.fin, fred);
+  if (tid == 0) {
+    *h.fin.arrive = 0;
+    *h.fin.pos = (*h.fin.pos + 1) % h.fin.capacity;
+    atomicAdd(h.fin.iter, 1);
+  }
+}
+
+}
diff --git a/gnndelete_amd/engine.py b/gnndelete_amd/engine.py
--- a/gnndelete_amd/engine.py
+++ b/gnndelete_amd/engine.py
@@ -143,6 +143,16 @@
 def plan_explicit_chain(facts, forms, covers, enabled=True, *, fold1, n_explicit):
     return bool(enabled and covers and fold1 and facts.mode == 'gcn' and not forms.rows_only and not facts.cache_layer1
                 and facts.h == 128 and facts.o == 64 and n_explicit > 0)
+
+
+def read_tail_hosted(env=None):
+    env = os.environ if env is None else env
+    return env.get('GD_TAIL_HOSTED') != '0'
+
+
+def plan_tail_hosted(facts, forms, enabled=True, *, fold1, fold2, wide, padded):
+    return bool(enabled and fold1 and fold2 and forms.tail and forms.chain1 and forms.fuse_wg2 and facts.mode == 'gcn'
+                and facts.loss_type == 'both_layerwise' and not forms.rows_only and wide and not padded)
 
 
 def _loss_coefficients(loss_type, alpha):
@@ -603,6 +613,11 @@
             self.facts, self.forms,
             self._fold1 and bool(lib.gd_rows_gemm_select_chain_covers(self.s1, int(self._idx1c.numel()), x.shape[1], self.h, self.o)),
             read_explicit_chain(), fold1=self._fold1, n_explicit=int(self._idx1c.numel()) if self._fold1 else 0)
+        self._tail_hosted = plan_tail_hosted(
+            self.facts, self.forms, read_tail_hosted(), fold1=self._fold1, fold2=self._fold2,
+            wide=ops.spmm_wide_form(self.o, n, self.o, self.o), padded=self._user_wd2 is not None)
+        if self._tail_hosted:
+            self._w1t = self._w1.t().contiguous()
         self._gat_r1 = None
         if self._mode == 'gat':
             w2_ = conv2.lin_src.weight.detach()
@@ -763,7 +778,8 @@
         elif self._mode in ('gcn', 'gin', 'sage'):
             idx, out, plan = (self.idx2, self._t2buf, self._plan2) if self._rows_only else (None, None, None)
             if self._mode == 'gcn':
-                self._spmm(False, self.graph.val, self._linear_relu_z1(c.lin.weight, idx, out), self.p2, c.bias, 0.0, plan=plan)
+                self._spmm(False, self.graph.val, self._linear_relu_z1(c.lin.weight, idx, out), self.p2, c.bias, 0.0, plan=plan,
+                           host=self._tail_host(1))
             elif self._mode == 'gin':
                 lin = c.nn
                 if lin.out_features > lin.in_features:
@@ -811,7 +827,7 @@
             else:
                 dt2, plan = (self._dt2_keep if chain else torch.empty(self.n, self.o, dtype=torch.float32, device=self.x.device)), None
             if self._mode == 'gcn':
-                self._spmm(True, g.val_t, self.dz2, dt2, None, 0.0, plan=plan)
+                self._spmm(True, g.val_t, self.dz2, dt2, None, 0.0, plan=plan, host=self._tail_host(2))
                 w2 = c.lin.weight
             else:
                 self._spmm(True, None, self.dz2, dt2, None, 1.0 + c.eps, plan=plan)
@@ -835,12 +851,36 @@
             ops.rank1_add2_(dt2, da_s, c.att_src, da_d, c.att_dst)
         ops.rows_gemm(dt2, self.idx1, w2, trans_w=False, out=self.dh, gate_bits=self.z1_pos)
 
-    def _spmm(self, transposed, val, x, y, bias, self_coef, x_self=None, plan=None):
+    def _spmm(self, transposed, val, x, y, bias, self_coef, x_self=None, plan=None, host=None):
         g = self.graph
         if transposed:
-            ops._spmm_raw(g.rowptr_t, g.col_t, val, x, bias, self_coef, self.n, plan or g.plan_t, out=y, x_self=x_self)
+            ops._spmm_raw(g.rowptr_t, g.col_t, val, x, bias, self_coef, self.n, plan or g.plan_t, out=y, x_self=x_self, host=host)
         else:
-            ops._spmm_raw(g.rowptr, g.col, val, x, bias, self_coef, self.n, plan or g.plan, out=y, x_self=x_self)
+            ops._spmm_raw(g.rowptr, g.col, val, x, bias, self_coef, self.n, plan or g.plan, out=y, x_self=x_self, host=host)
+
+    def step_stages(self):
+        if not (self._fold1 and self._fold2 and self._chain1 and self._tail and not self._rows_only):
+            return None
+        stages = ['spmm1'] + ([] if self._chain_expl else ['pre1_rest']) + ['del1_loss_wgrad1', 't2', 'spmm2', 'del2_loss_bwd', 'spmm2_t']
+        return stages + ([] if self._tail_hosted else ['tail'])
+
+    def _loss_partials(self):
+        p1, n1 = ((self._lp1, self._lp1_blocks + (self.t1.outside_blocks() if self._out1 else 0)) if self._fuse_loss1
+                  else (self.t1.partials, self.t1.n_partial_blocks()))
+        p2, n2 = ((self._lp2, self._lp2_blocks + (self.t2.outside_blocks() if self._out2 else 0)) if self._fuse_l2
+                  else (self.t2.partials, self.t2.n_partial_blocks()))
+        return p1, n1, p2, n2
+
+    def _tail_host(self, job):
+        if not self._tail_hosted:
+            return None
+        a1, a2 = self.adam1, self.adam2
+        p1, n1, p2, n2 = self._loss_partials()
+        return (ptr(self.ws1), ptr(self._cs1), self._lp1_blocks if job == 1 else 0, self.h, ptr(self._w1), ptr(self._w1t), ptr(self._b1),
+                ptr(self.g1), ptr(a1.param), ptr(a1.m), ptr(a1.v), ptr(self._wf), ptr(self._bf),
+                ptr(self.ws2), self._lp2_blocks if job == 2 else 0, self.o, self._tail_acc[1], ptr(self.g2), ptr(a2.param), ptr(a2.m),
+                ptr(a2.v), a1.lr, a1.betas[0], a1.betas[1], a1.eps,
+                ptr(p1), n1, ptr(p2), n2, ptr(self.hist), self.hist.shape[0], ptr(self.hist_pos), ptr(self.iter_ctr), ptr(self._arrive))
 
     def _wgrad(self, a_compact, g, g_idx, n_sel, out, accumulate, ws, adam=None, g_add=None, a_idx=None):
         d_a, d_b = a_compact.shape[1], g.shape[1]
@@ -932,11 +972,10 @@
                 self._wgrad(a1, self.dh, self.idx1, self.s1, self.g1, False, self.ws1, adam=self.adam1, a_idx=a1_idx)
             if lt != 'only1' and not self._fuse_l2 and not self._tail:
                 self.adam2.apply(self.g2)
-            p1, n1 = ((self._lp1, self._lp1_blocks + (self.t1.outside_blocks() if self._out1 else 0)) if self._fuse_loss1
-                      else (self.t1.partials, self.t1.n_partial_blocks()))
-            p2, n2 = ((self._lp2, self._lp2_blocks + (self.t2.outside_blocks() if self._out2 else 0)) if self._fuse_l2
-                      else (self.t2.partials, self.t2.n_partial_blocks()))
-            if self._tail:
+            p1, n1, p2, n2 = self._loss_partials()
+            if self._tail_hosted:
+                pass
+            elif self._tail:
                 a1, a2 = self.adam1, self.adam2
                 lib_ = _lib.lib()
                 nw1 = self._lp1_blocks if self._fuse_del1 else lib_.gd_rows_gemm_wgrad_blocks(self.s1)
diff --git a/gnndelete_amd/ops.py b/gnndelete_amd/ops.py
--- a/gnndelete_amd/ops.py
+++ b/gnndelete_amd/ops.py
@@ -26,7 +26,19 @@
 
 
 
-def _spmm_raw(rowptr, col, val, x, bias, self_coef, n_rows, plan=None, out=None, x_self=None, wide=True):
+def spmm_wide_form(d, x_rows, ld_x, ld_y, env=None):
+    env = os.environ if env is None else env
+    return bool(d == 64 and ld_x % 4 == 0 and x_rows < (1 << 24) and ld_x * 4 < (1 << 24) and ld_y * 4 < (1 << 24)
+                and x_rows * ld_x * 4 < (1 << 32) and x_rows * ld_y * 4 < (1 << 32) and env.get('GD_SPMM_TWO_LAUNCH') != '1'
+                and env.get('GD_SPMM_MULTIROW') != '0' and not env.get('GD_SPMM_D64_FORM'))
+
+
+def _no_host(host):
+    if host is not None:
+        raise _lib.GnnDeleteHipError('the step tail can only ride on the wide 64-float aggregation (gd_spmm_csr_onepass_wide_hosted_f32)')
+
+
+def _spmm_raw(rowptr, col, val, x, bias, self_coef, n_rows, plan=None, out=None, x_self=None, wide=True, host=None):
     d = x.shape[1]
     if x_self is not None:
         assert plan is not None and x_self.stride(0) == x.stride(0) and x_self.shape[1] == d
@@ -34,21 +46,23 @@
     if (plan is not None and d % 4 == 0 and d <= 1024 and x.stride(0) % 4 == 0 and x.data_ptr() % 16 == 0
             and os.environ.get('GD_SPMM_TWO_LAUNCH') != '1'):
         x_rows = max(int(x.shape[0]), int(y.shape[0]))
-        if (wide and d == 64 and x_rows < (1 << 24) and x.stride(0) * 4 < (1 << 24) and y.stride(0) * 4 < (1 << 24)
-                and x_rows * x.stride(0) * 4 < (1 << 32) and x_rows * y.stride(0) * 4 < (1 << 32)
-                and os.environ.get('GD_SPMM_MULTIROW') != '0' and not os.environ.get('GD_SPMM_D64_FORM')):
+        if wide and spmm_wide_form(d, x_rows, x.stride(0), y.stride(0)):
             items, n_items, bounds, tags = plan.onepass_wide(d)
-            check(_lib.lib().gd_spmm_csr_onepass_wide_f32(ptr(items), n_items, ptr(_wide_col(plan, col, tags)), ptr(val), ptr(x), x.stride(0),
-                                                          ptr(y), y.stride(0), ptr(bias), float(self_coef), ptr(x_self), d,
-                                                          int(col.shape[0]), x_rows, ptr(bounds), stream_ptr(x.device)),
-                  'gd_spmm_csr_onepass_wide_f32')
+            args = (ptr(items), n_items, ptr(_wide_col(plan, col, tags)), ptr(val), ptr(x), x.stride(0), ptr(y), y.stride(0), ptr(bias),
+                    float(self_coef), ptr(x_self), d, int(col.shape[0]), x_rows, ptr(bounds))
+            if host is not None:
+                check(_lib.lib().gd_spmm_csr_onepass_wide_hosted_f32(*args, *host, stream_ptr(x.device)), 'gd_spmm_csr_onepass_wide_hosted_f32')
+                return y
+            check(_lib.lib().gd_spmm_csr_onepass_wide_f32(*args, stream_ptr(x.device)), 'gd_spmm_csr_onepass_wide_f32')
             return y
+        _no_host(host)
         items, n_items, bounds = plan.onepass(d)
         check(_lib.lib().gd_spmm_csr_onepass_f32(ptr(items), n_items, ptr(col), ptr(val), ptr(x), x.stride(0), ptr(y),
                                                  y.stride(0), ptr(bias), float(self_coef), ptr(x_self), d, int(col.shape[0]),
                                                  max(int(x.shape[0]), int(y.shape[0])), ptr(bounds), stream_ptr(x.device)),
               'gd_spmm_csr_onepass_f32')
         return y
+    _no_host(host)
     if plan is not None and d % 4 == 0 and d <= 1024 and x.stride(0) % 4 == 0 and x.data_ptr() % 16 == 0:
         scratch = plan.scratch(d, x.device)
         check(_lib.lib().gd_spmm_csr_balanced_f32(ptr(plan.items), plan.n_items, ptr(plan.split), plan.n_split,
diff --git a/include/gnndelete_hip.h b/include/gnndelete_hip.h
--- a/include/gnndelete_hip.h
+++ b/include/gnndelete_hip.h
@@ -272,6 +272,14 @@
                            float* dw2, float* param2, float* exp_avg2, float* exp_avg_sq2, double lr, double beta1, double beta2,
                            double eps, const float* loss_partials1, int32_t n1, const float* loss_partials2, int32_t n2,
                            float* hist, int32_t capacity, int32_t* pos, int32_t* iter, int32_t* arrive, void* stream);
+int gd_spmm_csr_onepass_wide_hosted_f32(
+    const int32_t* items, int32_t n_items, const int32_t* col_tagged, const float* val, const float* x, int64_t ldx, float* y, int64_t ldy,
+    const float* bias, float self_coef, const float* x_self, int32_t d, int32_t nnz, int32_t x_rows, const int32_t* xcd_bounds,
+    const float* partials1_t, const float* colsum1, int32_t n_part1, int32_t d1, const float* w1, const float* w1_t, const float* b1,
+    float* dw1, float* param1, float* exp_avg1, float* exp_avg_sq1, float* w_fold, float* bias_fold, const float* partials2,
+    int32_t n_part2, int32_t d2, int32_t accumulate2, float* dw2, float* param2, float* exp_avg2, float* exp_avg_sq2, double lr,
+    double beta1, double beta2, double eps, const float* loss_partials1, int32_t n1, const float* loss_partials2, int32_t n2, float* hist,
+    int32_t capacity, int32_t* pos, int32_t* iter, int32_t* arrive, void* stream);
 
 
 int64_t gd_rowpair_mse_workspace(int32_t n_seg);
```

Measured after the change: 2182 iters/s (median of 6 runs). 2.0% higher.
